# rsjahnige/CRYSTALS-Kyber

Hardware: NVIDIA B200
Metric: ML-KEM-768 Encaps+Decaps ops/s (higher is better)
Workload: dtype u16/u64 integer

## Files before the change

crystals-kyber_b200/csrc/mlkem_b200.cu:

```cuda
#include "mlkem_kernels.cuh"

#include "../../include/mlkem_b200.h"

#include <algorithm>
#include <atomic>
#include <cstdio>
#include <cstdlib>
#include <cstring>
#include <mutex>
#include <vector>

namespace {

using namespace mlkem;

thread_local char tl_error[512] = "";
std::atomic<unsigned long long> g_launches{0};
int env_int(const char *name, int dflt) {
    const char *v = getenv(name);
    return v && *v ? atoi(v) : dflt;
}
constexpr int kSlots = 6;
constexpr int kDevSlots = 4;
constexpr int kHostSlots = 3;
constexpr int kMaxDevices = 64;
int initial_streams() {
    int v = env_int("MLKEM_B200_STREAMS", 0);
    return v < 1 ? kDevSlots : (v > kDevSlots ? kDevSlots : v);
}
std::atomic<int> g_streams{initial_streams()};
int warp_hash_max() {
    static const int v = env_int("MLKEM_B200_WARP_HASH_MAX", kWarpHashMaxItems);
    return v;
}

#define CU(call)                                                                                              \
    do {                                                                                                      \
        cudaError_t e_ = (call);                                                                              \
        if (e_ != cudaSuccess) {                                                                              \
            snprintf(tl_error, sizeof tl_error, "%s failed: %s (%s:%d)", #call, cudaGetErrorString(e_), __FILE__, __LINE__); \
            return MLKEM_B200_ERR_CUDA;                                                                       \
        }                                                                                                     \
    } while (0)

struct ProfEntry {
    const char *name;
    cudaEvent_t e0, e1;
};
std::atomic<int> g_profile{0};
std::mutex g_prof_mutex;
std::vector<ProfEntry> g_prof_entries;

inline void prof_begin(const char *name, cudaStream_t st, ProfEntry &pe, bool &on) {
    on = g_profile.load(std::memory_order_relaxed) != 0;
    if (!on) return;
    pe.name = name;
    cudaEventCreate(&pe.e0);
    cudaEventCreate(&pe.e1);
    cudaEventRecord(pe.e0, st);
}
inline void prof_end(cudaStream_t st, ProfEntry &pe, bool on) {
    if (!on) return;
    cudaEventRecord(pe.e1, st);
    std::lock_guard<std::mutex> lock(g_prof_mutex);
    g_prof_entries.push_back(pe);
}

#define LAUNCH(kernel, grid, block, smem, stream, ...)           \
    do {                                                         \
        auto kern_ = kernel;                                     \
        ProfEntry pe_;                                           \
        bool prof_on_;                                           \
        prof_begin(#kernel, (stream), pe_, prof_on_);            \
        kern_<<<(grid), (block), (smem), (stream)>>>(__VA_ARGS__); \
        prof_end((stream), pe_, prof_on_);                       \
        g_launches.fetch_add(1, std::memory_order_relaxed);      \
        CU(cudaGetLastError());                                  \
    } while (0)

inline unsigned cdiv(size_t a, size_t b) { return (unsigned)((a + b - 1) / b); }
inline unsigned warp_hash_grid(int n) { return cdiv((size_t)n, kWarpHashTPB / 32); }
inline unsigned warp_grid(size_t items, int warps_per_block) {
    size_t blocks = (items + warps_per_block - 1) / warps_per_block;
    const size_t cap = 148 * 16;
    return (unsigned)(blocks < cap ? blocks : cap);
}

unsigned bitrev7(unsigned r) {
    unsigned o = 0;
    for (int i = 0; i < 7; i++) o |= ((r >> i) & 1u) << (6 - i);
    return o;
}
unsigned pow17(unsigned e) {
    unsigned z = 1;
    while (e--) z = (z * 17u) % kQ;
    return z;
}
uint2 shoup_pair(unsigned w) { return make_uint2(w, (w << 16) / kQ); }
uint2 shoup_pair32(unsigned w) { return make_uint2(w, (unsigned)(((unsigned long long)w << 32) / kQ)); }

void build_tables(TwiddleTables &t, uint2 rc[24]) {
    for (unsigned i = 0; i < 128; i++) {
        t.zeta[i] = shoup_pair(pow17(bitrev7(i)));
        t.gamma[i] = shoup_pair(pow17(2 * bitrev7(i) + 1));
        t.gamma32[i] = shoup_pair32(t.gamma[i].x);
        t.zeta32[i] = shoup_pair32(t.zeta[i].x);
    }
    t.zeta_inv_last[0] = shoup_pair((t.zeta[1].x * 3303u) % kQ);
    t.zeta_inv_last[1] = shoup_pair(3303u);
    t.zeta_inv_last32[0] = shoup_pair32(t.zeta_inv_last[0].x);
    t.zeta_inv_last32[1] = shoup_pair32(3303u);
    uint8_t lfsr = 1;
    for (int round = 0; round < 24; round++) {
        unsigned long long c = 0;
        for (int j = 0; j <= 6; j++) {
            if (lfsr & 1) c |= 1ULL << ((1u << j) - 1);
            uint8_t hi = lfsr & 0x80;
            lfsr = (uint8_t)(lfsr << 1);
            if (hi) lfsr ^= 0x71;
        }
        rc[round] = make_uint2((unsigned)c, (unsigned)(c >> 32));
    }
}

struct DeviceCtx {
    bool ready = false;
    cudaStream_t stream[kSlots] = {};
    void *ws[kSlots] = {};
    size_t ws_bytes[kSlots] = {};
    void *io[kSlots] = {};
    size_t io_bytes[kSlots] = {};
    cudaEvent_t ev_fork = nullptr, ev_join[kSlots] = {}, ev_slot[kSlots] = {};
    void *misc = nullptr;
    size_t misc_bytes = 0;
    int host_group = 0;
    std::mutex call_mutex;
    std::mutex misc_mutex;
};
DeviceCtx g_ctx[kMaxDevices];
std::mutex g_mutex;

struct DeviceGuard {
    int prev = -1;
    bool changed = false;
    int enter(int d) {
        if (cudaGetDevice(&prev) != cudaSuccess) prev = -1;
        if (prev == d) return 0;
        CU(cudaSetDevice(d));
        changed = true;
        return 0;
    }
    ~DeviceGuard() {
        if (changed && prev >= 0) cudaSetDevice(prev);
    }
};

int ensure_buffer(void **p, size_t *have, size_t need, cudaEvent_t last_use = nullptr) {
    if (*have >= need) return 0;
    if (*p) {
        if (last_use) CU(cudaEventSynchronize(last_use));
        CU(cudaMemset(*p, 0, *have));
        CU(cudaFree(*p));
    }
    *p = nullptr;
    *have = 0;
    size_t want = need + need / 8;
    CU(cudaMalloc(p, want));
    *have = want;
    return 0;
}

template <class KernelT>
int allow_smem(KernelT kernel, size_t bytes) {
    CU(cudaFuncSetAttribute(kernel, cudaFuncAttributeMaxDynamicSharedMemorySize, (int)bytes));
    CU(cudaFuncSetAttribute(kernel, cudaFuncAttributePreferredSharedMemoryCarveout, cudaSharedmemCarveoutMaxShared));
    return 0;
}
template <class P>
int allow_smem_matvec() {
    const size_t b = matvec_smem_bytes<P>();
    if (int rc = allow_smem(k_sample_matvec<P, kModeKeyGen>, b)) return rc;
    if (int rc = allow_smem(k_sample_matvec<P, kModeEncrypt>, b)) return rc;
    if (int rc = allow_smem(k_sample_matvec<P, kModeEncryptCompare>, b)) return rc;
    if (int rc = allow_smem(k_sample_matvec_list<P, kModeKeyGen>, b)) return rc;
    if (int rc = allow_smem(k_sample_matvec_list<P, kModeEncrypt>, b)) return rc;
    if (int rc = allow_smem(k_sample_matvec_list<P, kModeEncryptCompare>, b)) return rc;
    return 0;
}

int acquire(const mlkem_b200_opts *o, int *dev, DeviceCtx **ctx, DeviceGuard &guard) {
    int d = o ? o->device : -1;
    if (d < 0) CU(cudaGetDevice(&d));
    if (d >= kMaxDevices) {
        snprintf(tl_error, sizeof tl_error, "device ordinal %d out of range", d);
        return MLKEM_B200_ERR_ARG;
    }
    if (int rc = guard.enter(d)) return rc;
    std::lock_guard<std::mutex> lock(g_mutex);
    DeviceCtx &c = g_ctx[d];
    if (!c.ready) {
        cudaStream_t st[kSlots] = {};
        cudaEvent_t ev[2 * kSlots + 1] = {};
        auto create = [&]() -> int {
            TwiddleTables t;
            uint2 rc[24];
            build_tables(t, rc);
            CU(cudaMemcpyToSymbol(c_tw, &t, sizeof t));
            CU(cudaMemcpyToSymbol(g_tw, &t, sizeof t));
            CU(cudaMemcpyToSymbol(c_keccak_rc, rc, sizeof rc));
            uint32_t pow2[32];
            for (int k = 0; k < 32; k++) pow2[k] = 1u << k;
            CU(cudaMemcpyToSymbol(c_pow2, pow2, sizeof pow2));
            for (int s = 0; s < kSlots; s++) CU(cudaStreamCreateWithFlags(&st[s], cudaStreamNonBlocking));
            for (int e = 0; e < 2 * kSlots + 1; e++) CU(cudaEventCreateWithFlags(&ev[e], cudaEventDisableTiming));
            if (int r = allow_smem_matvec<P512>()) return r;
            if (int r = allow_smem_matvec<P768>()) return r;
            if (int r = allow_smem_matvec<P1024>()) return r;
            if (int r = allow_smem(k_sample_ntt_batch, 128 * kSlotWords * 4)) return r;
            return 0;
        };
        if (int r = create()) {
            for (auto s_ : st)
                if (s_) cudaStreamDestroy(s_);
            for (auto e_ : ev)
                if (e_) cudaEventDestroy(e_);
            return r;
        }
        for (int s = 0; s < kSlots; s++) {
            c.stream[s] = st[s];
            c.ev_join[s] = ev[s];
            c.ev_slot[s] = ev[kSlots + s];
        }
        c.ev_fork = ev[2 * kSlots];
        c.ready = true;
    }
    *dev = d;
    *ctx = &c;
    return 0;
}

struct Arena {
    uint8_t *base;
    size_t off = 0;
    explicit Arena(void *p) : base(static_cast<uint8_t *>(p)) {}
    template <class T>
    T *take(size_t count) {
        off = (off + 255) & ~size_t(255);
        T *p = reinterpret_cast<T *>(base + off);
        off += count * sizeof(T);
        return p;
    }
};

template <class P>
constexpr size_t ws_bytes_per_item() {
    size_t kg = 64 + 2 * P::K * 512 + 4 * P::K;
    size_t enc = P::K * 512 + (P::K + 1) * 128 + 32 + 4 * P::K;
    size_t dec = enc + 32 + 64 + 4;
    size_t m = kg > dec ? kg : dec;
    return m + 64;
}
constexpr size_t kWsSlack = 16 * 256;


template <class P, int MODE>
int launch_matvec(cudaStream_t st, Arena &ws, MatvecArgs a) {
    constexpr int K = P::K;
    const size_t rows = (size_t)a.n * K, smem = matvec_smem_bytes<P>();
    const unsigned blocks = cdiv(rows, 32), list_grid = std::min<unsigned>(blocks, 148 * 4);
#ifdef MLKEM_B200_EXPERIMENT
    static const int env_exp = env_int("MLKEM_B200_EXPERIMENT", 0);
    a.experiment = env_exp;
#endif
    if (a.group_limit >= 168 && rows > 32) {
        a.defer_list = ws.take<int>(rows);
        a.defer_count = ws.take<int>(1);
        CU(cudaMemsetAsync(a.defer_count, 0, sizeof(int), st));
        LAUNCH((k_sample_matvec<P, MODE>), blocks, 32 * K, smem, st, a);
#ifdef MLKEM_B200_EXPERIMENT
        if (env_exp & 16) return 0;
#endif
        LAUNCH((k_sample_matvec_list<P, MODE>), list_grid, 32 * K, smem, st, a);
    } else {
        a.defer_list = nullptr;
        a.defer_count = nullptr;
        LAUNCH((k_sample_matvec_list<P, MODE>), list_grid, 32 * K, smem, st, a);
    }
    return 0;
}

template <class P>
int enqueue_encrypt(cudaStream_t st, Arena &ws, int n, const uint8_t *ek, size_t ek_stride, KeySel keys, const uint8_t *m,
                    const uint8_t *seed, size_t seed_stride, uint8_t *c, const uint8_t *cmp, uint32_t *flags, int group_limit, bool fips,
                    const uint16_t *matrix = nullptr) {
    constexpr int K = P::K;
    uint16_t *yhat = ws.take<uint16_t>((size_t)n * K * 256);
    uint32_t *codes = ws.take<uint32_t>((size_t)n * (K + 1) * 32);
    if (!fips) {
        LAUNCH((k_noise<P::ETA1, true>), dim3(cdiv(n, kNoiseTPB), K), kNoiseTPB, 0, st, n, seed, seed_stride, 0, yhat, (size_t)K * 256,
               (uint32_t *)nullptr, (size_t)0, (uint8_t *)nullptr, (size_t)0, 0);
        LAUNCH((k_noise<P::ETA2, false>), dim3(cdiv(n, kNoiseTPB), K + 1), kNoiseTPB, 0, st, n, seed, seed_stride, K, (uint16_t *)nullptr,
               (size_t)0, codes, (size_t)(K + 1) * 32, (uint8_t *)nullptr, (size_t)0, 0);
    } else {
        LAUNCH((k_noise<P::ETA1, true, kRateSha3_256>), dim3(cdiv(n, kNoiseTPB), K), kNoiseTPB, 0, st, n, seed, seed_stride, 0, yhat,
               (size_t)K * 256, (uint32_t *)nullptr, (size_t)0, (uint8_t *)nullptr, (size_t)0, 0);
        LAUNCH((k_noise<P::ETA2, false, kRateSha3_256>), dim3(cdiv(n, kNoiseTPB), K + 1), kNoiseTPB, 0, st, n, seed, seed_stride, K,
               (uint16_t *)nullptr, (size_t)0, codes, (size_t)(K + 1) * 32, (uint8_t *)nullptr, (size_t)0, 0);
    }
    MatvecArgs a{};
    a.n = n;
    a.group_limit = group_limit;
    a.rho = ek + 384 * K;
    a.rho_stride = ek_stride;
    a.keys = keys;
    a.vec = yhat;
    a.vec_stride = (size_t)K * 256;
    a.addc = codes;
    a.addc_stride = (size_t)(K + 1) * 32;
    a.out = c;
    a.out_stride = P::C;
    a.cmp = cmp;
    a.flags = flags;
    EncVArgs v{};
    v.n = n;
    v.ek = ek;
    v.ek_stride = ek_stride;
    v.keys = keys;
    v.yhat = yhat;
    v.yhat_stride = (size_t)K * 256;
    v.addc = codes;
    v.addc_stride = (size_t)(K + 1) * 32;
    v.m = m;
    v.c = c;
    v.c_stride = P::C;
    v.cmp = cmp;
    v.flags = flags;
    const unsigned tgrid = warp_grid((size_t)n * K, kMatTableTPB / 32);
    if (cmp) {
        if (matrix) LAUNCH((k_matvec_table<P, kModeEncryptCompare>), tgrid, kMatTableTPB, 0, st, a, matrix);
        else if (int rc = launch_matvec<P, kModeEncryptCompare>(st, ws, a)) return rc;
        LAUNCH((k_encrypt_v<P, true>), warp_grid(n, kWarpTPB / 32), kWarpTPB, 0, st, v);
    } else {
        if (matrix) LAUNCH((k_matvec_table<P, kModeEncrypt>), tgrid, kMatTableTPB, 0, st, a, matrix);
        else if (int rc = launch_matvec<P, kModeEncrypt>(st, ws, a)) return rc;
        LAUNCH((k_encrypt_v<P, false>), warp_grid(n, kWarpTPB / 32), kWarpTPB, 0, st, v);
    }
    return 0;
}

template <class P>
int enqueue_keygen(cudaStream_t st, Arena &ws, int n, const uint8_t *d, const uint8_t *z, uint8_t *ek, uint8_t *dk, int group_limit, bool fips) {
    constexpr int K = P::K;
    const bool full = z != nullptr;
    const size_t dk_stride = full ? P::DK : P::DKPKE;
    uint8_t *rs = ws.take<uint8_t>((size_t)n * 64);
    uint16_t *se = ws.take<uint16_t>((size_t)n * 2 * K * 256);
    LAUNCH(k_keygen_G, cdiv(n, kHashTPB), kHashTPB, 0, st, n, d, (uint32_t)K, rs, ek + 384 * K, (size_t)P::EK,
           full ? dk + 768 * K : (uint8_t *)nullptr, dk_stride);
    if (!fips)
        LAUNCH((k_noise<P::ETA1, true>), dim3(cdiv(n, kNoiseTPB), 2 * K), kNoiseTPB, 0, st, n, rs + 32, (size_t)64, 0, se, (size_t)2 * K * 256,
               (uint32_t *)nullptr, (size_t)0, dk, dk_stride, K);
    else
        LAUNCH((k_noise<P::ETA1, true, kRateSha3_256>), dim3(cdiv(n, kNoiseTPB), 2 * K), kNoiseTPB, 0, st, n, rs + 32, (size_t)64, 0, se,
               (size_t)2 * K * 256, (uint32_t *)nullptr, (size_t)0, dk, dk_stride, K);
    MatvecArgs a{};
    a.n = n;
    a.group_limit = group_limit;
    a.rho = rs;
    a.rho_stride = 64;
    a.vec = se;
    a.vec_stride = (size_t)2 * K * 256;
    a.add16 = se + K * 256;
    a.add16_stride = (size_t)2 * K * 256;
    a.out = ek;
    a.out_stride = P::EK;
    a.out2 = full ? dk + 384 * K : nullptr;
    a.out2_stride = dk_stride;
    if (int rc = launch_matvec<P, kModeKeyGen>(st, ws, a)) return rc;
    if (full && n <= warp_hash_max()) LAUNCH((k_keygen_H_warp<P>), warp_hash_grid(n), kWarpHashTPB, 0, st, n, ek, z, dk);
    else if (full) LAUNCH((k_keygen_H<P>), cdiv(n, kHashTPB), kHashTPB, 0, st, n, ek, z, dk);
    return 0;
}

template <class P>
int enqueue_encaps(cudaStream_t st, Arena &ws, int n, const uint8_t *ek, const uint8_t *m, uint8_t *c, uint8_t *Kout, int group_limit, bool fips) {
    uint8_t *r = ws.take<uint8_t>((size_t)n * 32);
    if (n <= warp_hash_max()) LAUNCH((k_encaps_HG_warp<P>), warp_hash_grid(n), kWarpHashTPB, 0, st, n, ek, m, Kout, r);
    else LAUNCH((k_encaps_HG<P>), cdiv(n, kHashTPB), kHashTPB, 0, st, n, ek, m, Kout, r);
    return enqueue_encrypt<P>(st, ws, n, ek, P::EK, KeySel{}, m, r, 32, c, nullptr, nullptr, group_limit, fips);
}

template <class P>
int enqueue_encaps_keyed(cudaStream_t st, Arena &ws, int n, const uint8_t *ek, size_t ek_stride, const uint8_t *hek, KeySel keys,
                         const uint8_t *m, uint8_t *c, uint8_t *Kout, int group_limit, bool fips, const uint16_t *matrix) {
    uint8_t *r = ws.take<uint8_t>((size_t)n * 32);
    LAUNCH(k_encaps_G_keyed, cdiv(n, kHashTPB), kHashTPB, 0, st, n, hek, keys, m, Kout, r);
    return enqueue_encrypt<P>(st, ws, n, ek, ek_stride, keys, m, r, 32, c, nullptr, nullptr, group_limit, fips, matrix);
}

template <class P>
int enqueue_decaps(cudaStream_t st, Arena &ws, int n, const uint8_t *dk, KeySel keys, const uint8_t *c, uint8_t *Kout, int group_limit, bool fips,
                   const uint16_t *matrix = nullptr) {
    constexpr int K = P::K;
    uint8_t *mp = ws.take<uint8_t>((size_t)n * 32);
    uint8_t *Kr = ws.take<uint8_t>((size_t)n * 64);
    uint32_t *flags = ws.take<uint32_t>((size_t)n);
    CU(cudaMemsetAsync(flags, 0, (size_t)n * 4, st));
    LAUNCH((k_decrypt<P>), warp_grid(n, kWarpTPB / 32), kWarpTPB, 0, st, n, dk, (size_t)P::DK, keys, c, mp);
    LAUNCH((k_decaps_G<P>), cdiv(n, kHashTPB), kHashTPB, 0, st, n, mp, dk, keys, Kr);
    if (int rc = enqueue_encrypt<P>(st, ws, n, dk + 384 * K, P::DK, keys, mp, Kr + 32, 64, nullptr, c, flags, group_limit, fips, matrix)) return rc;
    if (n <= warp_hash_max()) {
        if (!fips) LAUNCH((k_decaps_J_select_warp<P>), warp_hash_grid(n), kWarpHashTPB, 0, st, n, dk, keys, c, Kr, flags, Kout);
        else LAUNCH((k_decaps_J_select_warp<P, kRateSha3_256>), warp_hash_grid(n), kWarpHashTPB, 0, st, n, dk, keys, c, Kr, flags, Kout);
        return 0;
    }
    if (!fips) LAUNCH((k_decaps_J_select<P>), cdiv(n, kHashTPB), kHashTPB, 0, st, n, dk, keys, c, Kr, flags, Kout);
    else LAUNCH((k_decaps_J_select<P, kRateSha3_256>), cdiv(n, kHashTPB), kHashTPB, 0, st, n, dk, keys, c, Kr, flags, Kout);
    return 0;
}

struct Buf {
    const void *in;
    void *out;
    size_t item_bytes;
    bool cells = false;
};

int launch_narrow(cudaStream_t st, const void *cells, void *dense, size_t bytes) {
    const size_t nw = bytes / 4;
    if (nw) LAUNCH(k_cells_to_bytes, cdiv(nw, 256), 256, 0, st, nw, (const uint4 *)cells, (uint32_t *)dense);
    return 0;
}
int launch_widen(cudaStream_t st, const void *dense, void *cells, size_t bytes) {
    const size_t nw = bytes / 4;
    if (nw) LAUNCH(k_bytes_to_cells, cdiv(nw, 256), 256, 0, st, nw, (const uint32_t *)dense, (uint4 *)cells);
    return 0;
}

bool aligned16(const void *p) { return (reinterpret_cast<uintptr_t>(p) & 15) == 0; }

template <class Run>
int drive(const mlkem_b200_opts *o, size_t n, size_t ws_per_item, std::vector<Buf> bufs, Run run) {
    if (n == 0) return MLKEM_B200_OK;
    if (n > 0x7FFFFFFFull / 8) {
        snprintf(tl_error, sizeof tl_error, "batch too large");
        return MLKEM_B200_ERR_ARG;
    }
    for (auto &b : bufs)
        if (!b.in && !b.out) {
            snprintf(tl_error, sizeof tl_error, "NULL buffer");
            return MLKEM_B200_ERR_ARG;
        }
    int dev;
    DeviceCtx *ctx;
    DeviceGuard guard;
    if (int rc = acquire(o, &dev, &ctx, guard)) return rc;
    std::unique_lock<std::mutex> call_lock(ctx->call_mutex);
    const bool on_device = o && o->mem == MLKEM_B200_MEM_DEVICE;
    static const int env_chunk = env_int("MLKEM_B200_CHUNK", 0);
    static const int env_hchunk = env_int("MLKEM_B200_HOST_CHUNK", 0);
    static const int host_slots = std::min(kHostSlots, std::max(1, env_int("MLKEM_B200_HOST_SLOTS", kHostSlots)));
    size_t chunk = (o && o->chunk_items > 0) ? (size_t)o->chunk_items
                   : (on_device ? (env_chunk > 0 ? (size_t)env_chunk : (size_t)1 << 18) : (env_hchunk > 0 ? (size_t)env_hchunk : (size_t)1 << 16));
    if (chunk > ((size_t)1 << 26)) chunk = (size_t)1 << 26;
    if (chunk > n) chunk = n;
    const size_t nchunks = (n + chunk - 1) / chunk;
    std::vector<void *> ptrs(bufs.size());
    size_t cell_dense_per_item = 0;
    for (auto &b : bufs)
        if (b.cells) cell_dense_per_item += (b.item_bytes + 15) & ~size_t(15);

    if (on_device) {
        for (auto &b : bufs)
            if (!aligned16(b.in ? b.in : b.out)) {
                snprintf(tl_error, sizeof tl_error, "device pointers must be 16-byte aligned");
                return MLKEM_B200_ERR_ARG;
            }
        cudaStream_t st = static_cast<cudaStream_t>(o->stream);
        if (!(o && o->chunk_items > 0) && n >= ((size_t)1 << 16) && nchunks < 2 && g_streams.load() > 1) {
            chunk = ((n + 1) / 2 + 1023) & ~(size_t)1023;
        }
        const size_t nch = (n + chunk - 1) / chunk;
        int nstreams = g_streams.load();
        if (nstreams > kDevSlots) nstreams = kDevSlots;
        if ((size_t)nstreams > nch) nstreams = (int)nch;
        if (nstreams < 1) nstreams = 1;
        {
            std::lock_guard<std::mutex> lock(g_mutex);
            for (int k = 0; k < nstreams; k++)
                if (int rc = ensure_buffer(&ctx->ws[k], &ctx->ws_bytes[k], chunk * (ws_per_item + cell_dense_per_item) + kWsSlack + 256 * bufs.size(),
                                           ctx->ev_slot[k]))
                    return rc;
        }
        const bool fork = nstreams > 1;
        if (fork) CU(cudaEventRecord(ctx->ev_fork, st));
        for (int k = 0; k < nstreams; k++) {
            cudaStream_t sk = fork ? ctx->stream[k] : st;
            if (fork) CU(cudaStreamWaitEvent(sk, ctx->ev_fork, 0));
            CU(cudaStreamWaitEvent(sk, ctx->ev_slot[k], 0));
        }
        int rc = 0;
        for (size_t ci = 0; ci < nch && !rc; ci++) {
            size_t i0 = ci * chunk, cn = (i0 + chunk <= n) ? chunk : n - i0;
            const int k = fork ? (int)(ci % nstreams) : 0;
            cudaStream_t sk = fork ? ctx->stream[k] : st;
            Arena arena(ctx->ws[k]);
            for (size_t b = 0; b < bufs.size() && !rc; b++) {
                const uint8_t *base = static_cast<const uint8_t *>(bufs[b].in ? bufs[b].in : bufs[b].out);
                if (!bufs[b].cells) {
                    ptrs[b] = const_cast<uint8_t *>(base) + i0 * bufs[b].item_bytes;
                } else {
                    ptrs[b] = arena.take<uint8_t>(cn * bufs[b].item_bytes);
// ... 1187 lines not shown
```

crystals-kyber_b200/csrc/mlkem_device.cuh:

```cuda
#pragma once
#include <cuda_runtime.h>
#include <stdint.h>

namespace mlkem {

constexpr int kN = 256;
constexpr uint32_t kQ = 3329;
constexpr uint32_t kFullMask = 0xFFFFFFFFu;

struct TwiddleTables {
    uint2 zeta[128];
    uint2 zeta_inv_last[2];
    uint2 gamma[128];
    uint2 gamma32[128];
    uint2 zeta32[128];
    uint2 zeta_inv_last32[2];
};
__constant__ TwiddleTables c_tw;
__device__ TwiddleTables g_tw;
__constant__ uint2 c_keccak_rc[24];
__constant__ uint32_t c_pow2[32];
__device__ __forceinline__ uint32_t shl_fma(uint32_t x, int k) { return x * c_pow2[k]; }
__device__ __forceinline__ uint2 lane_zeta(int i) { return __ldg(&g_tw.zeta[i]); }
__device__ __forceinline__ uint2 lane_zeta32(int i) { return __ldg(&g_tw.zeta32[i]); }
__device__ __forceinline__ uint2 lane_gamma(int i) { return __ldg(&g_tw.gamma32[i]); }


__device__ __forceinline__ uint32_t mulhi(uint32_t a, uint32_t b) {
#ifndef MLKEM_B200_MULHI_WIDE
    return __umulhi(a, b);
#else
    [[maybe_unused]] uint32_t lo;
    uint32_t hi;
    asm volatile("{.reg .b64 t; mul.wide.u32 t, %2, %3; mov.b64 {%0, %1}, t;}" : "=r"(lo), "=r"(hi) : "r"(a), "r"(b));
    return hi;
#endif
}

__device__ __forceinline__ uint32_t mul_shoup(uint32_t a, uint2 w) {
    uint32_t qh = (a * w.y) >> 16;
    return a * w.x - qh * kQ;
}
__device__ __forceinline__ uint32_t mul_shoup_fma(uint32_t a, uint32_t w, uint32_t w32) {
    uint32_t qh = mulhi(a, w32);
    return a * w - qh * kQ;
}
constexpr bool kFmaPipe = true, kBalanced = false;
template <bool FMA>
__device__ __forceinline__ uint32_t mulz(uint32_t a, uint2 z) {
    return FMA ? mul_shoup_fma(a, z.x, z.y) : mul_shoup(a, z);
}
__device__ __forceinline__ uint32_t canon_fma(uint32_t x) { return x - mulhi(x, 1290168u) * kQ; }
__device__ __forceinline__ uint32_t barrett16(uint32_t x) {
    uint32_t qh = (x * 40317u) >> 27;
    return x - qh * kQ;
}
__device__ __forceinline__ uint32_t barrett32(uint32_t x) {
    uint32_t qh = mulhi(x, 1290167u);
    return x - qh * kQ;
}
__device__ __forceinline__ uint32_t csubq(uint32_t r) { return min(r, r - kQ); }
__device__ __forceinline__ uint32_t canon16(uint32_t x) { return csubq(barrett16(x)); }
__device__ __forceinline__ uint32_t canon32(uint32_t x) { return csubq(barrett32(x)); }

template <int D>
__device__ __forceinline__ uint32_t compress(uint32_t x) {
    if (D >= 12) return x;
    uint32_t t = (x << D) + 1664u;
    uint32_t qh = mulhi(t, 1290167u);
    uint32_t r = t - qh * kQ;
    qh += (r >= kQ);
    return qh & ((1u << D) - 1u);
}
template <int D>
__device__ __forceinline__ uint32_t compress_canon(uint32_t x) {
    static_assert(D == 1 || D == 4 || D == 5 || D == 10 || D == 11, "no verified constants for this d");
    constexpr uint32_t c = (D >= 10) ? 1664u : 1665u, M = (D >= 10) ? 1290168u : 1290167u;
    return mulhi(x * (1u << D) + c, M) & ((1u << D) - 1u);
}

template <int D>
__device__ __forceinline__ uint32_t compress_resid(uint32_t x) {
    static_assert(D == 1 || D == 4 || D == 5, "single multiply-high is not exact on residues for this d");
    return mulhi(x * (1u << D) + 1664u, 1290168u) & ((1u << D) - 1u);
}

template <int D>
__device__ __forceinline__ uint32_t decompress(uint32_t y) {
    if (D >= 12) return y;
    return (kQ * y + (1u << (D - 1))) >> D;
}

struct Lane {
    uint32_t lo, hi;
};

template <int R>
__device__ __forceinline__ Lane rotl64(Lane x) {
    Lane r = x;
    if constexpr (R == 32) {
        r.lo = x.hi;
        r.hi = x.lo;
    } else if constexpr (R > 0 && R < 32) {
        r.hi = __funnelshift_l(x.lo, x.hi, R);
        r.lo = __funnelshift_l(x.hi, x.lo, R);
    } else if constexpr (R > 32) {
        r.hi = __funnelshift_l(x.hi, x.lo, R - 32);
        r.lo = __funnelshift_l(x.lo, x.hi, R - 32);
    }
    return r;
}
__device__ __forceinline__ Lane xor3(Lane a, Lane b, Lane c) { return Lane{a.lo ^ b.lo ^ c.lo, a.hi ^ b.hi ^ c.hi}; }
__device__ __forceinline__ Lane xor5(Lane a, Lane b, Lane c, Lane d, Lane e) {
    return Lane{a.lo ^ b.lo ^ c.lo ^ d.lo ^ e.lo, a.hi ^ b.hi ^ c.hi ^ d.hi ^ e.hi};
}
__device__ __forceinline__ Lane chi3(Lane a, Lane b, Lane c) { return Lane{a.lo ^ (~b.lo & c.lo), a.hi ^ (~b.hi & c.hi)}; }

__device__ __forceinline__ void keccak_f1600(Lane a[25]) {
#pragma unroll 2
    for (int rnd = 0; rnd < 24; rnd++) {
        Lane c0 = xor5(a[0], a[5], a[10], a[15], a[20]), c1 = xor5(a[1], a[6], a[11], a[16], a[21]),
             c2 = xor5(a[2], a[7], a[12], a[17], a[22]), c3 = xor5(a[3], a[8], a[13], a[18], a[23]),
             c4 = xor5(a[4], a[9], a[14], a[19], a[24]);
        Lane r0 = rotl64<1>(c0), r1 = rotl64<1>(c1), r2 = rotl64<1>(c2), r3 = rotl64<1>(c3), r4 = rotl64<1>(c4);
#define MLKEM_TH(x, cm, rp)             \
    a[x] = xor3(a[x], cm, rp);          \
    a[x + 5] = xor3(a[x + 5], cm, rp);  \
    a[x + 10] = xor3(a[x + 10], cm, rp); \
    a[x + 15] = xor3(a[x + 15], cm, rp); \
    a[x + 20] = xor3(a[x + 20], cm, rp);
        MLKEM_TH(0, c4, r1) MLKEM_TH(1, c0, r2) MLKEM_TH(2, c1, r3) MLKEM_TH(3, c2, r4) MLKEM_TH(4, c3, r0)
#undef MLKEM_TH
        Lane b[25];
        b[0] = a[0];             b[10] = rotl64<1>(a[1]);   b[20] = rotl64<62>(a[2]);  b[5] = rotl64<28>(a[3]);   b[15] = rotl64<27>(a[4]);
        b[16] = rotl64<36>(a[5]); b[1] = rotl64<44>(a[6]);   b[11] = rotl64<6>(a[7]);   b[21] = rotl64<55>(a[8]);  b[6] = rotl64<20>(a[9]);
        b[7] = rotl64<3>(a[10]);  b[17] = rotl64<10>(a[11]); b[2] = rotl64<43>(a[12]);  b[12] = rotl64<25>(a[13]); b[22] = rotl64<39>(a[14]);
        b[23] = rotl64<41>(a[15]); b[8] = rotl64<45>(a[16]); b[18] = rotl64<15>(a[17]); b[3] = rotl64<21>(a[18]);  b[13] = rotl64<8>(a[19]);
        b[14] = rotl64<18>(a[20]); b[24] = rotl64<2>(a[21]); b[9] = rotl64<61>(a[22]);  b[19] = rotl64<56>(a[23]); b[4] = rotl64<14>(a[24]);
#pragma unroll
        for (int y = 0; y < 25; y += 5) {
#pragma unroll
            for (int x = 0; x < 5; x++) a[y + x] = chi3(b[y + x], b[y + (x + 1) % 5], b[y + (x + 2) % 5]);
        }
        uint2 rc = c_keccak_rc[rnd];
        a[0].lo ^= rc.x;
        a[0].hi ^= rc.y;
    }
}

__device__ __forceinline__ void keccak_zero(Lane a[25]) {
#pragma unroll
    for (int i = 0; i < 25; i++) a[i] = Lane{0u, 0u};
}

constexpr uint32_t kSfxHash = 0x06;
constexpr uint32_t kSfxXof = 0x1F;
constexpr int kRateShake128 = 21;
constexpr int kRateSha3_256 = 17;
constexpr int kRateSha3_512 = 9;

template <int RATE, typename F>
__device__ __forceinline__ void sponge_absorb_words(Lane a[25], int nwords, uint32_t sfx, F word) {
    keccak_zero(a);
    int base = 0;
    for (; base + RATE <= nwords; base += RATE) {
#pragma unroll
        for (int i = 0; i < RATE; i++) {
            Lane w = word(base + i);
            a[i].lo ^= w.lo;
            a[i].hi ^= w.hi;
        }
        keccak_f1600(a);
    }
    int rem = nwords - base;
#pragma unroll
    for (int i = 0; i < RATE; i++) {
        if (i < rem) {
            Lane w = word(base + i);
            a[i].lo ^= w.lo;
            a[i].hi ^= w.hi;
        } else if (i == rem) {
            a[i].lo ^= sfx;
        }
    }
    a[RATE - 1].hi ^= 0x80000000u;
    keccak_f1600(a);
}

__device__ __forceinline__ Lane load_lane(const uint8_t *p) {
    uint2 v = *reinterpret_cast<const uint2 *>(p);
    return Lane{v.x, v.y};
}
__device__ __forceinline__ void store_lane(uint8_t *p, Lane v) { *reinterpret_cast<uint2 *>(p) = make_uint2(v.lo, v.hi); }

struct WarpSponge {
    int s5, s10, s15, s20;
    int xm, xp;
    int pi;
    int c1, c2;
    uint32_t shift;
    bool swap, first;
};
__device__ __forceinline__ WarpSponge warp_sponge_init(int lane) {
    constexpr uint32_t kRho[7] = {0u | 1u << 8 | 62u << 16 | 28u << 24,  27u | 36u << 8 | 44u << 16 | 6u << 24,  55u | 20u << 8 | 3u << 16 | 10u << 24,
                                  43u | 25u << 8 | 39u << 16 | 41u << 24, 45u | 15u << 8 | 21u << 16 | 8u << 24, 18u | 2u << 8 | 61u << 16 | 56u << 24,
                                  14u};
    WarpSponge w;
    const bool act = lane < 25;
    const int x = lane % 5, y = lane / 5;
    w.s5 = act ? (lane + 5) % 25 : lane;
    w.s10 = act ? (lane + 10) % 25 : lane;
    w.s15 = act ? (lane + 15) % 25 : lane;
    w.s20 = act ? (lane + 20) % 25 : lane;
    w.xm = act ? (x + 4) % 5 : lane;
    w.xp = act ? (x + 1) % 5 : lane;
    w.pi = act ? (x + 3 * y) % 5 + 5 * x : lane;
    w.c1 = act ? 5 * y + (x + 1) % 5 : lane;
    w.c2 = act ? 5 * y + (x + 2) % 5 : lane;
    uint32_t word = 0;
#pragma unroll
    for (int k = 0; k < 7; k++) word = (lane >> 2) == k ? kRho[k] : word;
    const uint32_t rot = act ? (word >> (8 * (lane & 3))) & 63u : 0u;
    w.shift = rot & 31u;
    w.swap = (rot & 32u) != 0;
    w.first = lane == 0;
    return w;
}
__device__ __forceinline__ Lane shfl_lane(Lane v, int src) {
    return Lane{__shfl_sync(kFullMask, v.lo, src), __shfl_sync(kFullMask, v.hi, src)};
}
__device__ __forceinline__ void keccak_f1600_warp(Lane &a, const WarpSponge &w) {
#pragma unroll 2
    for (int rnd = 0; rnd < 24; rnd++) {
        const Lane c = xor5(a, shfl_lane(a, w.s5), shfl_lane(a, w.s10), shfl_lane(a, w.s15), shfl_lane(a, w.s20));
        a = xor3(a, shfl_lane(c, w.xm), rotl64<1>(shfl_lane(c, w.xp)));
        const uint32_t lo = w.swap ? a.hi : a.lo, hi = w.swap ? a.lo : a.hi;
        a.hi = __funnelshift_l(lo, hi, w.shift);
        a.lo = __funnelshift_l(hi, lo, w.shift);
        const Lane b = shfl_lane(a, w.pi);
        a = chi3(b, shfl_lane(b, w.c1), shfl_lane(b, w.c2));
        const uint2 rc = c_keccak_rc[rnd];
        a.lo ^= w.first ? rc.x : 0u;
        a.hi ^= w.first ? rc.y : 0u;
    }
}
template <int RATE, typename F>
__device__ __forceinline__ Lane warp_sponge_absorb_words(int lane, const WarpSponge &w, int nwords, uint32_t sfx, F word) {
    Lane a{0u, 0u};
    int base = 0;
    for (; base + RATE <= nwords; base += RATE) {
        if (lane < RATE) {
            const Lane v = word(base + lane);
            a.lo ^= v.lo;
            a.hi ^= v.hi;
        }
        keccak_f1600_warp(a, w);
    }
    const int rem = nwords - base;
    if (lane < rem) {
        const Lane v = word(base + lane);
        a.lo ^= v.lo;
        a.hi ^= v.hi;
    } else if (lane == rem) {
        a.lo ^= sfx;
    }
    if (lane == RATE - 1) a.hi ^= 0x80000000u;
    keccak_f1600_warp(a, w);
    return a;
}

constexpr int kScratchU16 = 256;
__device__ __forceinline__ int sidx(int c) { return c ^ (((c >> 6) & 3) << 3); }
__device__ __forceinline__ int idxA(int lane, int r) { return lane + 32 * r; }
__device__ __forceinline__ int idxB(int lane, int r) { return ((lane >> 2) << 5) | (r << 2) | (lane & 3); }
__device__ __forceinline__ int idxC(int lane, int r) { return 8 * lane + r; }

struct LaneTwiddles {
    uint2 z16;
    uint2 z8[2];
    uint2 z4[4];
    uint2 z2[2];
};
template <bool FMA = false>
__device__ __forceinline__ uint2 lane_z(int i) { return FMA ? lane_zeta32(i) : lane_zeta(i); }
template <bool FMA = false>
__device__ __forceinline__ uint2 uniform_z(int i) { return FMA ? c_tw.zeta32[i] : c_tw.zeta[i]; }
template <bool FMA = false>
__device__ __forceinline__ void load_lane_twiddles(LaneTwiddles &t, int lane) {
    int g = lane >> 2;
    t.z16 = lane_z<FMA>(8 + g);
#pragma unroll
    for (int i = 0; i < 2; i++) t.z8[i] = lane_z<FMA>(16 + 2 * g + i);
#pragma unroll
    for (int i = 0; i < 4; i++) t.z4[i] = lane_z<FMA>(32 + 4 * g + i);
#pragma unroll
    for (int i = 0; i < 2; i++) t.z2[i] = lane_z<FMA>(64 + 2 * lane + i);
}
template <bool FMA = false>
__device__ __forceinline__ void load_lane_twiddles_inv(LaneTwiddles &t, int lane) {
    int g = lane >> 2;
    t.z16 = lane_z<FMA>(15 - g);
#pragma unroll
    for (int i = 0; i < 2; i++) t.z8[i] = lane_z<FMA>(31 - (2 * g + i));
#pragma unroll
    for (int i = 0; i < 4; i++) t.z4[i] = lane_z<FMA>(63 - (4 * g + i));
#pragma unroll
    for (int i = 0; i < 2; i++) t.z2[i] = lane_z<FMA>(127 - (2 * lane + i));
}

__device__ __forceinline__ void store_scratch_A(const uint32_t x[8], uint16_t *s, int lane) {
#pragma unroll
    for (int r = 0; r < 8; r++) s[sidx(idxA(lane, r))] = (uint16_t)x[r];
}
__device__ __forceinline__ void load_scratch_A(uint32_t x[8], const uint16_t *s, int lane) {
#pragma unroll
    for (int r = 0; r < 8; r++) x[r] = s[sidx(idxA(lane, r))];
}
__device__ __forceinline__ void store_scratch_B(const uint32_t x[8], uint16_t *s, int lane) {
#pragma unroll
    for (int r = 0; r < 8; r++) s[sidx(idxB(lane, r))] = (uint16_t)x[r];
}
__device__ __forceinline__ void load_scratch_B(uint32_t x[8], const uint16_t *s, int lane) {
#pragma unroll
    for (int r = 0; r < 8; r++) x[r] = s[sidx(idxB(lane, r))];
}
__device__ __forceinline__ uint4 pack_pairs(const uint32_t x[8]) {
    return make_uint4(x[0] + x[1] * 65536u, x[2] + x[3] * 65536u, x[4] + x[5] * 65536u, x[6] + x[7] * 65536u);
}
__device__ __forceinline__ void unpack_pairs(uint4 v, uint32_t x[8]) {
    x[0] = v.x & 0xFFFFu; x[1] = v.x >> 16; x[2] = v.y & 0xFFFFu; x[3] = v.y >> 16;
    x[4] = v.z & 0xFFFFu; x[5] = v.z >> 16; x[6] = v.w & 0xFFFFu; x[7] = v.w >> 16;
}
__device__ __forceinline__ void store_scratch_C(const uint32_t x[8], uint16_t *s, int lane) {
    *reinterpret_cast<uint4 *>(s + sidx(8 * lane)) = pack_pairs(x);
}
__device__ __forceinline__ void load_scratch_C(uint32_t x[8], const uint16_t *s, int lane) {
    unpack_pairs(*reinterpret_cast<const uint4 *>(s + sidx(8 * lane)), x);
}

template <bool FMA = false>
__device__ __forceinline__ void ct_bfly(uint32_t &a, uint32_t &b, uint2 z) {
    uint32_t t = mulz<FMA>(b, z);
    b = a - t + 2 * kQ;
    a = a + t;
}

template <bool FMA = false>
__device__ __forceinline__ void ntt_warp(uint32_t x[8], uint16_t *scratch, int lane, const LaneTwiddles &tw) {
#pragma unroll
    for (int r = 0; r < 4; r++) ct_bfly<FMA>(x[r], x[r + 4], uniform_z<FMA>(1));
#pragma unroll
    for (int h = 0; h < 2; h++)
#pragma unroll
        for (int r = 0; r < 2; r++) ct_bfly<FMA>(x[4 * h + r], x[4 * h + r + 2], uniform_z<FMA>(2 + h));
#pragma unroll
    for (int h = 0; h < 4; h++) ct_bfly<FMA>(x[2 * h], x[2 * h + 1], uniform_z<FMA>(4 + h));
    store_scratch_A(x, scratch, lane);
    __syncwarp();
    load_scratch_B(x, scratch, lane);
    __syncwarp();
#pragma unroll
    for (int r = 0; r < 4; r++) ct_bfly<FMA>(x[r], x[r + 4], tw.z16);
#pragma unroll
    for (int h = 0; h < 2; h++)
#pragma unroll
        for (int r = 0; r < 2; r++) ct_bfly<FMA>(x[4 * h + r], x[4 * h + r + 2], tw.z8[h]);
#pragma unroll
    for (int h = 0; h < 4; h++) ct_bfly<FMA>(x[2 * h], x[2 * h + 1], tw.z4[h]);
    store_scratch_B(x, scratch, lane);
    __syncwarp();
    load_scratch_C(x, scratch, lane);
    __syncwarp();
#pragma unroll
    for (int h = 0; h < 2; h++)
#pragma unroll
        for (int r = 0; r < 2; r++) ct_bfly<FMA>(x[4 * h + r], x[4 * h + r + 2], tw.z2[h]);
#pragma unroll
    for (int r = 0; r < 8; r++) x[r] = FMA ? canon_fma(x[r]) : canon16(x[r]);
}

__device__ __forceinline__ void ct_bfly_exact(uint32_t &a, uint32_t &b, uint2 z) {
    const uint32_t t = csubq(mul_shoup(b, z)), lo = a;
    b = lo >= t ? lo - t : kQ - (t - lo);
    a = canon16(lo + t);
}
__device__ __forceinline__ void ntt_warp_exact(uint32_t x[8], uint16_t *scratch, int lane) {
    LaneTwiddles tw;
    load_lane_twiddles<false>(tw, lane);
#pragma unroll
    for (int r = 0; r < 4; r++) ct_bfly_exact(x[r], x[r + 4], uniform_z<false>(1));
#pragma unroll
    for (int h = 0; h < 2; h++)
#pragma unroll
        for (int r = 0; r < 2; r++) ct_bfly_exact(x[4 * h + r], x[4 * h + r + 2], uniform_z<false>(2 + h));
#pragma unroll
    for (int h = 0; h < 4; h++) ct_bfly_exact(x[2 * h], x[2 * h + 1], uniform_z<false>(4 + h));
    store_scratch_A(x, scratch, lane);
    __syncwarp();
    load_scratch_B(x, scratch, lane);
    __syncwarp();
#pragma unroll
    for (int r = 0; r < 4; r++) ct_bfly_exact(x[r], x[r + 4], tw.z16);
#pragma unroll
    for (int h = 0; h < 2; h++)
#pragma unroll
        for (int r = 0; r < 2; r++) ct_bfly_exact(x[4 * h + r], x[4 * h + r + 2], tw.z8[h]);
#pragma unroll
    for (int h = 0; h < 4; h++) ct_bfly_exact(x[2 * h], x[2 * h + 1], tw.z4[h]);
    store_scratch_B(x, scratch, lane);
    __syncwarp();
    load_scratch_C(x, scratch, lane);
    __syncwarp();
#pragma unroll
    for (int h = 0; h < 2; h++)
#pragma unroll
        for (int r = 0; r < 2; r++) ct_bfly_exact(x[4 * h + r], x[4 * h + r + 2], tw.z2[h]);
}

template <bool FMA = false>
__device__ __forceinline__ void gs_bfly(uint32_t &a, uint32_t &b, uint2 z, uint32_t bias) {
    uint32_t t = a;
    a = t + b;
    b = mulz<FMA>(b - t + bias, z);
}

template <bool FMA = false, bool CANON = true>
__device__ __forceinline__ void intt_warp(uint32_t x[8], uint16_t *scratch, int lane, const LaneTwiddles &tw) {
#pragma unroll
    for (int h = 0; h < 2; h++)
#pragma unroll
        for (int r = 0; r < 2; r++) gs_bfly<FMA>(x[4 * h + r], x[4 * h + r + 2], tw.z2[h], (FMA ? 3 : 2) * kQ);
    store_scratch_C(x, scratch, lane);
    __syncwarp();
    load_scratch_B(x, scratch, lane);
    __syncwarp();
#pragma unroll
    for (int h = 0; h < 4; h++) {
        gs_bfly<FMA>(x[2 * h], x[2 * h + 1], tw.z4[h], (FMA ? 5 : 3) * kQ);
        x[2 * h] = FMA ? barrett32(x[2 * h]) : barrett16(x[2 * h]);
    }
#pragma unroll
    for (int h = 0; h < 2; h++)
#pragma unroll
        for (int r = 0; r < 2; r++) gs_bfly<FMA>(x[4 * h + r], x[4 * h + r + 2], tw.z8[h], 2 * kQ);
#pragma unroll
    for (int r = 0; r < 4; r++) gs_bfly<FMA>(x[r], x[r + 4], tw.z16, 4 * kQ);
    store_scratch_B(x, scratch, lane);
    __syncwarp();
    load_scratch_A(x, scratch, lane);
    __syncwarp();
#pragma unroll
    for (int h = 0; h < 4; h++) {
        gs_bfly<FMA>(x[2 * h], x[2 * h + 1], uniform_z<FMA>(7 - h), 8 * kQ);
        x[2 * h] = FMA ? barrett32(x[2 * h]) : barrett16(x[2 * h]);
    }
#pragma unroll
    for (int h = 0; h < 2; h++)
#pragma unroll
        for (int r = 0; r < 2; r++) gs_bfly<FMA>(x[4 * h + r], x[4 * h + r + 2], uniform_z<FMA>(3 - h), 2 * kQ);
    const uint2 zs = FMA ? c_tw.zeta_inv_last32[1] : c_tw.zeta_inv_last[1], zl = FMA ? c_tw.zeta_inv_last32[0] : c_tw.zeta_inv_last[0];
#pragma unroll
    for (int r = 0; r < 4; r++) {
        uint32_t t = x[r];
        x[r] = mulz<FMA>(t + x[r + 4], zs);
        x[r + 4] = mulz<FMA>(x[r + 4] - t + 4 * kQ, zl);
        if (CANON) {
            x[r] = csubq(x[r]);
            x[r + 4] = csubq(x[r + 4]);
        }
    }
}

__device__ __forceinline__ void basemul_acc(uint32_t &acc0, uint32_t &acc1, uint32_t a0, uint32_t a1, uint32_t b0,
                                            uint32_t b1, uint2 gamma) {
    uint32_t a1g = mul_shoup_fma(a1, gamma.x, gamma.y);
    acc0 += a0 * b0 + a1g * b1;
    acc1 += a0 * b1 + a1 * b0;
}

template <int D>
__device__ __forceinline__ void pack8(const uint32_t v[8], uint8_t *dst) {
    constexpr int NW = (8 * D + 31) / 32;
    uint32_t w[NW];
#pragma unroll
    for (int k = 0; k < NW; k++) {
        uint32_t acc = 0;
#pragma unroll
        for (int i = 0; i < 8; i++) {
            const int off = D * i - 32 * k;
            if (off >= 0 && off < 32) acc += v[i] * (1u << off);
            else if (off < 0 && off + D > 0) acc += v[i] >> (-off);
        }
        w[k] = acc;
    }
    if (D % 4 == 0) {
#pragma unroll
        for (int k = 0; k < NW; k++) reinterpret_cast<uint32_t *>(dst)[k] = w[k];
    } else if (D % 2 == 0) {
#pragma unroll
        for (int h = 0; h < D / 2; h++) reinterpret_cast<uint16_t *>(dst)[h] = (uint16_t)(w[h >> 1] >> (16 * (h & 1)));
    } else {
#pragma unroll
        for (int b8 = 0; b8 < D; b8++) dst[b8] = (uint8_t)(w[b8 >> 2] >> (8 * (b8 & 3)));
    }
}
template <int D>
__device__ __forceinline__ void unpack8(const uint8_t *row, int lane, uint32_t v[8]) {
    const uint32_t *w = reinterpret_cast<const uint32_t *>(row);
    const int bit = 8 * D * lane, wi = bit >> 5, s = bit & 31;
    constexpr int NA = (8 * D + 31) / 32;
    uint32_t raw[NA + 1], a[NA + 1];
#pragma unroll
    for (int k = 0; k <= NA; k++) raw[k] = ((8 * D) % 32 == 0 && k == NA) ? 0u : w[wi + k];
#pragma unroll
    for (int k = 0; k < NA; k++) a[k] = ((8 * D) % 32 == 0) ? raw[k] : __funnelshift_r(raw[k], raw[k + 1], s);
    a[NA] = 0;
#pragma unroll
    for (int i = 0; i < 8; i++) {
        const int o = D * i, k = o >> 5, sh = o & 31;
        uint32_t f = (sh + D <= 32) ? (a[k] >> sh) : __funnelshift_r(a[k], a[k + 1], sh);
        v[i] = f & ((1u << D) - 1u);
    }
}

template <int D>
__device__ __forceinline__ uint32_t unpack1(const uint8_t *src, int c) {
    if (D == 1) return (src[c >> 3] >> (c & 7)) & 1u;
    if (D == 4) return (src[c >> 1] >> ((c & 1) * 4)) & 15u;
    const int bit = D * c, byte = bit >> 3, sh = bit & 7;
    uint32_t w = (uint32_t)src[byte];
    if (sh + D > 8) w |= (uint32_t)src[byte + 1] << 8;
    if (D > 9 && sh + D > 16) w |= (uint32_t)src[byte + 2] << 16;
    return (w >> sh) & ((1u << D) - 1u);
}

template <int S>
__device__ __forceinline__ uint32_t shr_fma(uint32_t x) {
    return mulhi(x, 1u << (32 - S));
}
#ifndef MLKEM_B200_NIBBLE_ALU
__device__ __forceinline__ uint32_t nibble_fma(uint32_t w, uint32_t sel) { return shr_fma<28>(w * sel); }
__device__ __forceinline__ uint32_t nibble_weight(int j) { return 1u << (28 - 4 * j); }
#else
__device__ __forceinline__ uint32_t nibble_fma(uint32_t w, uint32_t sel) { return (w >> sel) & 15u; }
__device__ __forceinline__ uint32_t nibble_weight(int j) { return 4 * j; }
#endif

__device__ __forceinline__ uint32_t noise_code_to_coeff(uint32_t code) {
    return csubq(code + (kQ - 3));
}
__device__ __forceinline__ uint32_t add_noise_code(uint32_t x, uint32_t code) {
    return csubq(csubq(x + code + (kQ - 3)));
}

}
```

crystals-kyber_b200/csrc/mlkem_kernels.cuh:

```cuda
#pragma once
#include "mlkem_device.cuh"

namespace mlkem {

template <int K_, int ETA1_, int ETA2_, int DU_, int DV_>
struct ParamSet {
    static constexpr int K = K_, ETA1 = ETA1_, ETA2 = ETA2_, DU = DU_, DV = DV_;
    static constexpr int EK = 384 * K + 32;
    static constexpr int DKPKE = 384 * K;
    static constexpr int DK = 768 * K + 96;
    static constexpr int C1ROW = 32 * DU;
    static constexpr int C2 = 32 * DV;
    static constexpr int C = C1ROW * K + C2;
};
using P512 = ParamSet<2, 3, 2, 10, 4>;
using P768 = ParamSet<3, 2, 2, 10, 4>;
using P1024 = ParamSet<4, 2, 2, 11, 5>;

struct KeySel {
    const uint32_t *index;
    uint32_t base, nkeys;
};
__device__ __forceinline__ size_t key_row(const KeySel &k, int item) {
    if (k.index) return min(__ldg(k.index + item), k.nkeys - 1u);
// ... 115 lines not shown
__global__ void __launch_bounds__(kHashTPB) k_hash_ek_table(int n, const uint8_t *__restrict__ ek, size_t ek_stride, uint8_t *__restrict__ hek) {
    int i = blockIdx.x * blockDim.x + threadIdx.x;
    if (i >= n) return;
    Lane h[4];
    hash_H_ek<P>(ek + ek_stride * i, h);
#pragma unroll
    for (int w = 0; w < 4; w++) store_lane(hek + 32 * (size_t)i + 8 * w, h[w]);
}

template <class P>
__global__ void __launch_bounds__(kHashTPB) k_check_dk_hash(int n, const uint8_t *__restrict__ dk, int *__restrict__ status) {
    int i = blockIdx.x * blockDim.x + threadIdx.x;
    if (i >= n) return;
    const uint8_t *base = dk + (size_t)P::DK * i;
    Lane h[4];
    hash_H_ek<P>(base + 384 * P::K, h);
    uint32_t diff = 0;
#pragma unroll
    for (int w = 0; w < 4; w++) {
        Lane s = load_lane(base + 768 * P::K + 32 + 8 * w);
        diff |= (s.lo ^ h[w].lo) | (s.hi ^ h[w].hi);
    }
    status[i] = diff ? -5 : 0;
}

template <class P>
__global__ void __launch_bounds__(kHashTPB) k_check_ek_modulus(int n, const uint8_t *__restrict__ ek, int *__restrict__ status) {
    int i = blockIdx.x * blockDim.x + threadIdx.x;
    if (i >= n) return;
    const uint32_t *w = reinterpret_cast<const uint32_t *>(ek + (size_t)P::EK * i);
    uint32_t bad = 0;
    for (int t = 0; t < 96 * P::K; t += 3) {
        uint32_t w0 = __ldg(w + t), w1 = __ldg(w + t + 1), w2 = __ldg(w + t + 2);
        uint32_t c[8] = {w0 & 0xFFF, (w0 >> 12) & 0xFFF, (w0 >> 24) | ((w1 & 0xF) << 8), (w1 >> 4) & 0xFFF,
                         (w1 >> 16) & 0xFFF, (w1 >> 28) | ((w2 & 0xFF) << 4), (w2 >> 8) & 0xFFF, w2 >> 20};
#pragma unroll
        for (int k = 0; k < 8; k++) bad |= (c[k] >= kQ);
    }
    status[i] = bad ? -4 : 0;
}

__global__ void __launch_bounds__(kHashTPB) k_mask_keys(int n, const int *__restrict__ status, uint8_t *__restrict__ K) {
    int i = blockIdx.x * blockDim.x + threadIdx.x;
    if (i >= n) return;
    if (status[i] != 0) {
        uint4 zero = make_uint4(0, 0, 0, 0);
        reinterpret_cast<uint4 *>(K + 32 * (size_t)i)[0] = zero;
        reinterpret_cast<uint4 *>(K + 32 * (size_t)i)[1] = zero;
    }
}

template <class P>
__global__ void __launch_bounds__(kHashTPB) k_decaps_G(int n, const uint8_t *__restrict__ mprime, const uint8_t *__restrict__ dk, KeySel keys,
                                                       uint8_t *__restrict__ Kr) {
    int i = blockIdx.x * blockDim.x + threadIdx.x;
    if (i >= n) return;
    Lane h[4], mm[4], a[25];
    const uint8_t *hp = dk + (size_t)P::DK * key_row(keys, i) + 768 * P::K + 32;
#pragma unroll
    for (int w = 0; w < 4; w++) {
        mm[w] = load_lane(mprime + 32 * (size_t)i + 8 * w);
        h[w] = load_lane(hp + 8 * w);
    }
    hash_G_64(a, mm, h);
#pragma unroll
    for (int w = 0; w < 8; w++) store_lane(Kr + 64 * (size_t)i + 8 * w, a[w]);
}

template <class P, int RATE = kRateShake128>
__global__ void __launch_bounds__(kHashTPB) k_decaps_J_select(int n, const uint8_t *__restrict__ dk, KeySel keys, const uint8_t *__restrict__ c,
                                                              const uint8_t *__restrict__ Kr, const uint32_t *__restrict__ flags,
                                                              uint8_t *__restrict__ Kout) {
    int i = blockIdx.x * blockDim.x + threadIdx.x;
    if (i >= n) return;
    const uint8_t *z = dk + (size_t)P::DK * key_row(keys, i) + 768 * P::K + 64;
    const uint8_t *ci = c + (size_t)P::C * i;
    Lane a[25];
    sponge_absorb_words<RATE>(a, 4 + P::C / 8, kSfxXof,
                              [&](int w) { return w < 4 ? load_lane(z + 8 * w) : load_lane(ci + 8 * (w - 4)); });
    uint32_t mask = flags[i] ? 0xFFFFFFFFu : 0u;
#pragma unroll
    for (int w = 0; w < 4; w++) {
        Lane kp = load_lane(Kr + 64 * (size_t)i + 8 * w);
        Lane o{(a[w].lo & mask) | (kp.lo & ~mask), (a[w].hi & mask) | (kp.hi & ~mask)};
        store_lane(Kout + 32 * (size_t)i + 8 * w, o);
    }
}

constexpr int kWarpHashTPB = 128;
constexpr int kWarpHashMaxItems = 1024;

template <class P>
__device__ __forceinline__ Lane warp_hash_H_ek(const uint8_t *ek, int lane, const WarpSponge &w) {
    return warp_sponge_absorb_words<kRateSha3_256>(lane, w, P::EK / 8, kSfxHash, [&](int i) { return load_lane(ek + 8 * i); });
}
__device__ __forceinline__ Lane warp_hash_G_64(const uint8_t *x, Lane y03, int lane, const WarpSponge &w) {
    const Lane y = shfl_lane(y03, (lane - 4) & 31);
    Lane a{0u, 0u};
    if (lane < 4) a = load_lane(x + 8 * lane);
    else if (lane < 8) a = y;
    else if (lane == 8) a = Lane{kSfxHash, 0x80000000u};
    keccak_f1600_warp(a, w);
    return a;
}

template <class P>
__global__ void __launch_bounds__(kWarpHashTPB) k_keygen_H_warp(int n, const uint8_t *__restrict__ ek, const uint8_t *__restrict__ z,
                                                                uint8_t *__restrict__ dk) {
    const int lane = threadIdx.x & 31, i = blockIdx.x * (kWarpHashTPB / 32) + (threadIdx.x >> 5);
    if (i >= n) return;
    const WarpSponge w = warp_sponge_init(lane);
    const Lane h = warp_hash_H_ek<P>(ek + (size_t)P::EK * i, lane, w);
    uint8_t *tail = dk + (size_t)P::DK * i + 768 * P::K + 32;
    if (lane < 4) store_lane(tail + 8 * lane, h);
    else if (lane < 8) store_lane(tail + 8 * lane, load_lane(z + 32 * (size_t)i + 8 * (lane - 4)));
}

template <class P>
__global__ void __launch_bounds__(kWarpHashTPB) k_encaps_HG_warp(int n, const uint8_t *__restrict__ ek, const uint8_t *__restrict__ m,
                                                                 uint8_t *__restrict__ Kout, uint8_t *__restrict__ r) {
    const int lane = threadIdx.x & 31, i = blockIdx.x * (kWarpHashTPB / 32) + (threadIdx.x >> 5);
    if (i >= n) return;
    const WarpSponge w = warp_sponge_init(lane);
    const Lane h = warp_hash_H_ek<P>(ek + (size_t)P::EK * i, lane, w);
    const Lane a = warp_hash_G_64(m + 32 * (size_t)i, h, lane, w);
    if (lane < 4) store_lane(Kout + 32 * (size_t)i + 8 * lane, a);
    else if (lane < 8) store_lane(r + 32 * (size_t)i + 8 * (lane - 4), a);
}

template <class P>
__global__ void __launch_bounds__(kWarpHashTPB) k_check_dk_hash_warp(int n, const uint8_t *__restrict__ dk, int *__restrict__ status) {
    const int lane = threadIdx.x & 31, i = blockIdx.x * (kWarpHashTPB / 32) + (threadIdx.x >> 5);
    if (i >= n) return;
    const WarpSponge w = warp_sponge_init(lane);
    const uint8_t *base = dk + (size_t)P::DK * i;
    const Lane h = warp_hash_H_ek<P>(base + 384 * P::K, lane, w);
    bool diff = false;
    if (lane < 4) {
        const Lane s = load_lane(base + 768 * P::K + 32 + 8 * lane);
        diff = ((s.lo ^ h.lo) | (s.hi ^ h.hi)) != 0;
    }
    const bool any = __any_sync(kFullMask, diff);
    if (lane == 0) status[i] = any ? -5 : 0;
}

template <class P, int RATE = kRateShake128>
__global__ void __launch_bounds__(kWarpHashTPB) k_decaps_J_select_warp(int n, const uint8_t *__restrict__ dk, KeySel keys, const uint8_t *__restrict__ c,
                                                                       const uint8_t *__restrict__ Kr, const uint32_t *__restrict__ flags,
                                                                       uint8_t *__restrict__ Kout) {
    const int lane = threadIdx.x & 31, i = blockIdx.x * (kWarpHashTPB / 32) + (threadIdx.x >> 5);
    if (i >= n) return;
    const WarpSponge w = warp_sponge_init(lane);
    const uint8_t *z = dk + (size_t)P::DK * key_row(keys, i) + 768 * P::K + 64;
    const uint8_t *ci = c + (size_t)P::C * i;
    const Lane a = warp_sponge_absorb_words<RATE>(lane, w, 4 + P::C / 8, kSfxXof,
                                                  [&](int t) { return t < 4 ? load_lane(z + 8 * t) : load_lane(ci + 8 * (t - 4)); });
    const uint32_t mask = flags[i] ? 0xFFFFFFFFu : 0u;
    if (lane < 4) {
        const Lane kp = load_lane(Kr + 64 * (size_t)i + 8 * lane);
        store_lane(Kout + 32 * (size_t)i + 8 * lane, Lane{(a.lo & mask) | (kp.lo & ~mask), (a.hi & mask) | (kp.hi & ~mask)});
    }
}

template <int RATE, int OUTW>
__global__ void __launch_bounds__(kHashTPB) k_hash_words(int n, const uint8_t *__restrict__ in, int nwords, uint32_t sfx,
                                                         uint8_t *__restrict__ out) {
    int i = blockIdx.x * blockDim.x + threadIdx.x;
    if (i >= n) return;
    const uint8_t *p = in + (size_t)nwords * 8 * i;
    Lane a[25];
    sponge_absorb_words<RATE>(a, nwords, sfx, [&](int w) { return load_lane(p + 8 * w); });
#pragma unroll
    for (int w = 0; w < OUTW; w++) store_lane(out + (size_t)OUTW * 8 * i + 8 * w, a[w]);
}

__global__ void __launch_bounds__(kHashTPB) k_sponge_padded(int n, const uint8_t *__restrict__ padded, int nblocks, int rl,
                                                            uint8_t *__restrict__ out, int out_bytes) {
    int i = blockIdx.x * blockDim.x + threadIdx.x;
    if (i >= n) return;
    const uint8_t *p = padded + (size_t)i * nblocks * rl * 8;
    Lane a[25];
    keccak_zero(a);
    for (int b = 0; b < nblocks; b++) {
#pragma unroll
        for (int l = 0; l < 25; l++)
            if (l < rl) {
                Lane w = load_lane(p + ((size_t)b * rl + l) * 8);
                a[l].lo ^= w.lo;
                a[l].hi ^= w.hi;
            }
        keccak_f1600(a);
    }
    const int out_stride = (out_bytes + 7) & ~7;
    uint8_t *o = out + (size_t)i * out_stride;
    int done = 0;
    while (done < out_bytes) {
        int take = min(rl * 8, out_bytes - done);
#pragma unroll
        for (int l = 0; l < 25; l++)
            if (l * 8 < take) store_lane(o + done + l * 8, a[l]);
        done += take;
        if (done < out_bytes) keccak_f1600(a);
    }
}


__device__ __forceinline__ uint32_t cbd2_word(uint32_t w) {
    uint32_t t = w - ((w >> 1) & 0x55555555u);
    uint32_t x = t & 0x33333333u, y = (t >> 2) & 0x33333333u;
    return x + (0x33333333u - y);
}
__device__ __forceinline__ uint32_t cbd3_chunk(uint32_t c24) {
    uint32_t t = (c24 & 0x249249u) + ((c24 >> 1) & 0x249249u) + ((c24 >> 2) & 0x249249u);
    uint32_t out = 0;
#pragma unroll
    for (int m = 0; m < 4; m++) {
        uint32_t x = (t >> (6 * m)) & 7u, y = (t >> (6 * m + 3)) & 7u;
        out |= (x + 3u - y) << (4 * m);
    }
    return out;
}
__device__ __forceinline__ void cbd3_words(uint32_t w0, uint32_t w1, uint32_t w2, uint32_t &o0, uint32_t &o1) {
    uint32_t c0 = w0 & 0xFFFFFFu, c1 = (w0 >> 24) | ((w1 & 0xFFFFu) << 8), c2 = (w1 >> 16) | ((w2 & 0xFFu) << 16), c3 = w2 >> 8;
    o0 = cbd3_chunk(c0) | (cbd3_chunk(c1) << 16);
    o1 = cbd3_chunk(c2) | (cbd3_chunk(c3) << 16);
}

template <int ETA, int RATE, typename PUT>
__device__ __forceinline__ void prf_cbd_codes(const Lane seed[4], uint32_t nonce, PUT put) {
    Lane a[25];
    keccak_zero(a);
#pragma unroll
    for (int w = 0; w < 4; w++) a[w] = seed[w];
    a[4].lo = nonce | (kSfxXof << 8);
    a[RATE - 1].hi ^= 0x80000000u;
    keccak_f1600(a);
    if (ETA == 2) {
#pragma unroll
        for (int l = 0; l < 16; l++) {
            put(2 * l, cbd2_word(a[l].lo));
            put(2 * l + 1, cbd2_word(a[l].hi));
        }
    } else {
        constexpr int W1 = 2 * RATE;
        constexpr int G1 = W1 / 3;
        uint32_t o0, o1;
#pragma unroll
        for (int g = 0; g < G1; g++) {
            const int w = 3 * g;
            uint32_t w0 = (w & 1) ? a[w >> 1].hi : a[w >> 1].lo, w1 = ((w + 1) & 1) ? a[(w + 1) >> 1].hi : a[(w + 1) >> 1].lo,
                     w2 = ((w + 2) & 1) ? a[(w + 2) >> 1].hi : a[(w + 2) >> 1].lo;
            cbd3_words(w0, w1, w2, o0, o1);
            put(2 * g, o0);
            put(2 * g + 1, o1);
        }
        constexpr int LEFT = W1 - 3 * G1;
        uint32_t carry = 0;
        if (LEFT) carry = ((W1 - 1) & 1) ? a[(W1 - 1) >> 1].hi : a[(W1 - 1) >> 1].lo;
        keccak_f1600(a);
        int next = 0;
        if (LEFT) {
            cbd3_words(carry, a[0].lo, a[0].hi, o0, o1);
            put(2 * G1, o0);
            put(2 * G1 + 1, o1);
            next = 2;
        }
#pragma unroll
        for (int g = G1 + (LEFT ? 1 : 0); g < 16; g++) {
            const int w = next + 3 * (g - G1 - (LEFT ? 1 : 0));
            uint32_t w0 = (w & 1) ? a[w >> 1].hi : a[w >> 1].lo, w1 = ((w + 1) & 1) ? a[(w + 1) >> 1].hi : a[(w + 1) >> 1].lo,
                     w2 = ((w + 2) & 1) ? a[(w + 2) >> 1].hi : a[(w + 2) >> 1].lo;
            cbd3_words(w0, w1, w2, o0, o1);
            put(2 * g, o0);
            put(2 * g + 1, o1);
        }
    }
}

__device__ __forceinline__ void store_layoutC_global(const uint32_t x[8], int lane, uint16_t *dst) {
    reinterpret_cast<uint4 *>(dst)[lane] = pack_pairs(x);
}
__device__ __forceinline__ void load_layoutC_global(uint32_t x[8], int lane, const uint16_t *src) {
    unpack_pairs(__ldg(reinterpret_cast<const uint4 *>(src) + lane), x);
}

template <int ETA, bool NTT_OUT, int RATE = kRateShake128>
__global__ void __launch_bounds__(kNoiseTPB) k_noise(int n, const uint8_t *__restrict__ seeds, size_t seed_stride, int nonce0,
                                                     uint16_t *__restrict__ out16, size_t out16_stride,
                                                     uint32_t *__restrict__ outc, size_t outc_stride,
                                                     uint8_t *__restrict__ enc12, size_t enc12_stride, int enc12_polys) {
    __shared__ uint32_t s_codes[NTT_OUT ? kNoiseTPB * 33 : 1];
    __shared__ __align__(16) uint16_t s_scratch[NTT_OUT ? (kNoiseTPB / 32) * kScratchU16 : 2];
    const int p = blockIdx.y;
    const int item = blockIdx.x * kNoiseTPB + threadIdx.x;
    Lane seed[4];
#pragma unroll
    for (int w = 0; w < 4; w++) seed[w] = item < n ? load_lane(seeds + seed_stride * item + 8 * w) : Lane{0u, 0u};
    if (NTT_OUT) {
        uint32_t *mine = s_codes + 33 * threadIdx.x;
        prf_cbd_codes<ETA, RATE>(seed, (uint32_t)(nonce0 + p), [&](int w, uint32_t v) { mine[w] = v; });
        __syncwarp();
        const int lane = threadIdx.x & 31, warp = threadIdx.x >> 5;
        uint16_t *scratch = s_scratch + warp * kScratchU16;
        LaneTwiddles tw;
        load_lane_twiddles<kFmaPipe>(tw, lane);
        const uint32_t pw = nibble_weight(lane & 7);
        for (int t = 0; t < 32; t++) {
            int it = blockIdx.x * kNoiseTPB + warp * 32 + t;
            if (it >= n) break;
            const uint32_t *codes = s_codes + 33 * (warp * 32 + t) + (lane >> 3);
            uint32_t x[8];
#pragma unroll
            for (int r = 0; r < 8; r++) x[r] = nibble_fma(codes[4 * r], pw) + (kQ - 3);
            ntt_warp<kFmaPipe>(x, scratch, lane, tw);
            store_layoutC_global(x, lane, out16 + out16_stride * it + 256 * p);
            if (p < enc12_polys) {
                uint32_t *row = reinterpret_cast<uint32_t *>(enc12 + enc12_stride * it + 384 * p) + 3 * lane;
                row[0] = x[0] | (x[1] << 12) | (x[2] << 24);
                row[1] = (x[2] >> 8) | (x[3] << 4) | (x[4] << 16) | (x[5] << 28);
                row[2] = (x[5] >> 4) | (x[6] << 8) | (x[7] << 20);
            }
        }
    } else {
        if (item >= n) return;
        uint32_t buf[32];
        prf_cbd_codes<ETA, RATE>(seed, (uint32_t)(nonce0 + p), [&](int w, uint32_t v) { buf[w] = v; });
        uint4 *dst = reinterpret_cast<uint4 *>(outc + outc_stride * item + 32 * p);
#pragma unroll
        for (int v = 0; v < 8; v++) dst[v] = make_uint4(buf[4 * v], buf[4 * v + 1], buf[4 * v + 2], buf[4 * v + 3]);
    }
}

template <bool CHECKED>
__device__ __forceinline__ void parse_block(const Lane a[25], uint32_t &addr, uint32_t end_addr) {
#pragma unroll
    for (int ch = 0; ch < 7; ch++) {
        const uint32_t w[7] = {a[3 * ch].lo, a[3 * ch].hi, a[3 * ch + 1].lo, a[3 * ch + 1].hi, a[3 * ch + 2].lo, a[3 * ch + 2].hi, 0u};
#pragma unroll
        for (int m = 0; m < 16; m++) {
            const int bit = 12 * m, wi = bit >> 5, sh = bit & 31;
            uint32_t t;
            if (sh == 20) t = w[wi];
            else if (sh < 20) t = w[wi] * (1u << (20 - sh));
            else t = __funnelshift_r(w[wi], w[wi + 1], sh - 20);
            bool ok = t < (kQ << 20);
            if (CHECKED) ok = ok && (addr < end_addr);
            uint32_t d;
            asm("mul.hi.u32 %0, %1, 4096;" : "=r"(d) : "r"(t));
            if (ok) {
                asm volatile("st.shared.u16 [%0], %1;" ::"r"(addr), "h"((uint16_t)d) : "memory");
                addr += 2;
            }
        }
    }
}

__device__ __forceinline__ void mask_groups(Lane a[25], int usable) {
    const int cut = 24 * max(usable, 0);
#pragma unroll
    for (int k = 0; k < 42; k++) {
        const int lo = 32 * k;
        uint32_t m = cut <= lo ? 0xFFFFFFFFu : (cut >= lo + 32 ? 0u : (0xFFFFFFFFu << (cut - lo)));
        if (k & 1) a[k >> 1].hi |= m;
        else a[k >> 1].lo |= m;
    }
}

__device__ __forceinline__ void sample_ntt_thread(const Lane rho[4], uint32_t &b32, uint32_t &b33, uint16_t *slot, bool active,
                                                  int group_limit) {
    Lane a[25];
    const uint32_t base = (uint32_t)__cvta_generic_to_shared(slot), end_addr = base + 2 * kN;
    uint32_t addr = active ? base : end_addr;
    int groups_left = 0;
    bool need_init = true;
    while (__any_sync(kFullMask, addr < end_addr)) {
        if (need_init) {
            keccak_zero(a);
#pragma unroll
            for (int w = 0; w < 4; w++) a[w] = rho[w];
            a[4].lo = (b32 & 0xFFu) | ((b33 & 0xFFu) << 8) | (kSfxXof << 16);
            a[kRateShake128 - 1].hi ^= 0x80000000u;
            groups_left = group_limit;
            need_init = false;
        }
        keccak_f1600(a);
        const bool running = addr < end_addr;
        if (__any_sync(kFullMask, running && groups_left < 56)) {
            if (running && groups_left < 56) mask_groups(a, groups_left);
        }
        if (__all_sync(kFullMask, addr + 2 * 112 <= end_addr)) parse_block<false>(a, addr, end_addr);
        else parse_block<true>(a, addr, end_addr);
        groups_left -= 56;
        if (groups_left <= 0 && addr < end_addr) {
            b32 = (b32 + 1) & 0xFFu;
            b33 = (b33 + 1) & 0xFFu;
            addr = base;
            need_init = true;
        }
    }
}

#ifdef MLKEM_B200_EXPERIMENT
#define MLKEM_CHECK_SLOT_STORE(st, lim) \
    if ((st) + 512 < end_addr || (st) > (lim)) __trap();
#else
#define MLKEM_CHECK_SLOT_STORE(st, lim)
#endif
template <bool CHECKED>
__device__ __forceinline__ void parse_chunk3(const uint32_t w[7], uint32_t &addr, uint32_t end_addr) {
#ifndef MLKEM_B200_PARSE_ALU_ADDR
    const uint32_t one = c_pow2[0], two = c_pow2[1];
#endif
#pragma unroll
    for (int m = 0; m < 16; m++) {
        const int bit = 12 * m, wi = bit >> 5, sh = bit & 31;
        uint32_t t;
        if (sh == 20) t = w[wi];
        else if (sh < 20) t = shl_fma(w[wi], 20 - sh);
        else t = __funnelshift_r(w[wi], w[wi + 1], sh - 20);
        const bool ok = t < (kQ << 20);
        MLKEM_CHECK_SLOT_STORE(addr, CHECKED ? end_addr : end_addr - 2)
        asm volatile("st.shared.u16 [%0], %1;" ::"r"(addr), "h"((uint16_t)(t >> 20)) : "memory");
#ifndef MLKEM_B200_PARSE_ALU_ADDR
        if (CHECKED)
            asm volatile("{.reg .pred p; setp.lt.u32 p, %1, %2; setp.lt.and.u32 p, %0, %3, p; @p mad.lo.u32 %0, %4, %5, %0;}"
                         : "+r"(addr) : "r"(t), "r"(kQ << 20), "r"(end_addr), "r"(one), "r"(two));
        else
            asm volatile("{.reg .pred p; setp.lt.u32 p, %1, %2; @p mad.lo.u32 %0, %3, %4, %0;}" : "+r"(addr) : "r"(t), "r"(kQ << 20), "r"(one), "r"(two));
        (void)ok;
#else
        if (CHECKED) {
            if (ok && addr < end_addr) addr += 2;
        } else {
            if (ok) addr += 2;
        }
#endif
    }
}
template <bool CHECKED>
__device__ __forceinline__ void parse_block3(const Lane a[25], uint32_t &addr, uint32_t end_addr) {
#pragma unroll
    for (int ch = 0; ch < 7; ch++) {
        const uint32_t w[7] = {a[3 * ch].lo, a[3 * ch].hi, a[3 * ch + 1].lo, a[3 * ch + 1].hi, a[3 * ch + 2].lo, a[3 * ch + 2].hi, 0u};
        parse_chunk3<CHECKED>(w, addr, end_addr);
    }
}
__device__ __forceinline__ bool sample_ntt_three_blocks(const Lane rho[4], uint32_t b32, uint32_t b33, uint16_t *slot, int experiment = 0) {
    Lane a[25];
    const uint32_t base = (uint32_t)__cvta_generic_to_shared(slot), end_addr = base + 2 * kN;
    uint32_t addr = base;
    keccak_zero(a);
#pragma unroll
    for (int w = 0; w < 4; w++) a[w] = rho[w];
    a[4].lo = (b32 & 0xFFu) | ((b33 & 0xFFu) << 8) | (kSfxXof << 16);
    a[kRateShake128 - 1].hi ^= 0x80000000u;
#pragma unroll 1
    for (int blk = 0; blk < 3; blk++) {
        keccak_f1600(a);
#ifdef MLKEM_B200_EXPERIMENT
        if (experiment & 2) {
            addr += a[0].lo & 2;
            continue;
        }
#endif
        if (blk < 2) parse_block3<false>(a, addr, end_addr);
        else parse_block3<true>(a, addr, end_addr);
    }
    return addr >= end_addr;
}

enum MatvecMode { kModeKeyGen = 0, kModeEncrypt = 1, kModeEncryptCompare = 2 };

struct MatvecArgs {
    int n;
    int group_limit;
    const uint8_t *rho;
    size_t rho_stride;
    KeySel keys;
    const uint16_t *vec;
    size_t vec_stride;
    const uint16_t *add16;
    size_t add16_stride;
    const uint32_t *addc;
    size_t addc_stride;
    uint8_t *out;
    size_t out_stride;
    uint8_t *out2;
    size_t out2_stride;
    const uint8_t *cmp;
    uint32_t *flags;
    int *defer_list;
    int *defer_count;
#ifdef MLKEM_B200_EXPERIMENT
    int experiment;
#endif
};

constexpr int kMatvecWarpBytes = 512 + 384;
template <class P>
__host__ __device__ constexpr size_t matvec_slots_bytes() {
    return ((size_t)32 * P::K * kSlotWords * 4 + 15) & ~(size_t)15;
}
template <class P>
constexpr size_t matvec_smem_bytes() {
    return matvec_slots_bytes<P>() + (size_t)P::K * kMatvecWarpBytes + 32 * 4 + 32 * P::K;
}

struct MatvecLaneConsts {
    uint2 gam[4];
    LaneTwiddles tw;
    uint32_t pw;
};
template <int MODE>
__device__ __forceinline__ void matvec_load_consts(MatvecLaneConsts &c, int lane) {
#pragma unroll
    for (int r = 0; r < 4; r++) c.gam[r] = lane_gamma(lane + 32 * r);
    if (MODE != kModeKeyGen) load_lane_twiddles_inv<kFmaPipe>(c.tw, lane);
    c.pw = nibble_weight(lane & 7);
}
template <class P>
struct MatvecOperands {
    static constexpr int kCmpWords = (8 * P::DU + 31) / 32;
    uint32_t v[8 * P::K], cw[8], cmp[kCmpWords], ev[4];
};
template <class P, int MODE>
__device__ __forceinline__ void matvec_prefetch(MatvecOperands<P> &o, const MatvecArgs &g, int gg, int lane) {
    constexpr int K = P::K;
    if (gg < 0) return;
    const int item = gg / K, row = gg - item * K;
    const uint16_t *vec = g.vec + g.vec_stride * item;
#pragma unroll
    for (int j = 0; j < K; j++)
#pragma unroll
        for (int r = 0; r < 4; r++) {
            int t = lane + 32 * r;
            o.v[8 * j + 2 * r] = __ldg(vec + 256 * j + 2 * t);
            o.v[8 * j + 2 * r + 1] = __ldg(vec + 256 * j + 2 * t + 1);
        }
    if (MODE == kModeEncryptCompare) {
        const uint32_t *cw = reinterpret_cast<const uint32_t *>(g.cmp + g.out_stride * item + (size_t)P::C1ROW * row);
#pragma unroll
        for (int i = 0; i < MatvecOperands<P>::kCmpWords; i++) o.cmp[i] = (lane + 32 * i < 8 * P::DU) ? __ldg(cw + lane + 32 * i) : 0u;
    }
    if (MODE != kModeKeyGen) {
        const uint32_t *codes = g.addc + g.addc_stride * item + 32 * row + (lane >> 3);
#pragma unroll
        for (int r = 0; r < 8; r++) o.cw[r] = __ldg(codes + 4 * r);
    } else {
        const uint32_t *ev = reinterpret_cast<const uint32_t *>(g.add16 + g.add16_stride * item + 256 * row);
#pragma unroll
        for (int r = 0; r < 4; r++) o.ev[r] = __ldg(ev + lane + 32 * r);
    }
}

template <class P, int MODE>
__device__ __forceinline__ void matvec_row_tail(const MatvecArgs &g, int item, int row, uint32_t acc[8], const uint32_t cw8[8],
                                                const uint32_t *cmpw, const uint32_t ev4[4], uint16_t *scratch, uint8_t *stage, int lane,
                                                const LaneTwiddles &tw, uint32_t pw) {
    constexpr int kCmpWords = MatvecOperands<P>::kCmpWords;
    int nwords;
    if (MODE == kModeKeyGen) {
#pragma unroll
        for (int r = 0; r < 4; r++) {
            int t = lane + 32 * r;
            uint32_t e = ev4[r];
            uint32_t c0 = csubq(canon32(acc[2 * r]) + (e & 0xFFFFu)), c1 = csubq(canon32(acc[2 * r + 1]) + (e >> 16));
            uint32_t v = c0 | (c1 << 12);
            stage[3 * t] = (uint8_t)v;
            stage[3 * t + 1] = (uint8_t)(v >> 8);
            stage[3 * t + 2] = (uint8_t)(v >> 16);
        }
        nwords = 96;
    } else {
        uint32_t *sw = reinterpret_cast<uint32_t *>(scratch);
#pragma unroll
        for (int r = 0; r < 4; r++) {
            int t = lane + 32 * r;
            sw[sidx(2 * t) >> 1] = barrett32(acc[2 * r]) + barrett32(acc[2 * r + 1]) * 65536u;
        }
        __syncwarp();
        uint32_t x[8];
        load_scratch_C(x, scratch, lane);
        __syncwarp();
        intt_warp<kFmaPipe, false>(x, scratch, lane, tw);
#pragma unroll
        for (int r = 0; r < 8; r++) {
            uint32_t y = x[r] + nibble_fma(cw8[r], pw) + (kQ - 3);
            x[r] = compress_canon<P::DU>(canon_fma(y));
        }
        store_scratch_A(x, scratch, lane);
        __syncwarp();
        load_scratch_C(x, scratch, lane);
        pack8<P::DU>(x, stage + P::DU * lane);
        nwords = 8 * P::DU;
    }
    __syncwarp();
    const uint32_t *stw = reinterpret_cast<const uint32_t *>(stage);
    const size_t row_off = (MODE == kModeKeyGen ? 384 : P::C1ROW) * (size_t)row;
    if (MODE == kModeEncryptCompare) {
        uint32_t d = 0;
#pragma unroll
        for (int i = 0; i < kCmpWords; i++)
            if (lane + 32 * i < nwords) d |= stw[lane + 32 * i] ^ cmpw[i];
        d = __any_sync(kFullMask, d != 0) ? 1u : 0u;
        if (lane == 0) atomicOr(g.flags + item, d);
    } else {
        uint32_t *ow = reinterpret_cast<uint32_t *>(g.out + g.out_stride * item + row_off);
        for (int w = lane; w < nwords; w += 32) ow[w] = stw[w];
        if (MODE == kModeKeyGen && g.out2) {
            uint32_t *ow2 = reinterpret_cast<uint32_t *>(g.out2 + g.out2_stride * item + row_off);
            for (int w = lane; w < nwords; w += 32) ow2[w] = stw[w];
        }
    }
    __syncwarp();
}

template <class P, int MODE>
__device__ __forceinline__ void matvec_finish_rows(const MatvecArgs &g, uint32_t *s_slots, const int *s_gg, int lane, int warp,
                                                   const MatvecLaneConsts &lc, MatvecOperands<P> &nx) {
    constexpr int K = P::K;
    uint8_t *warp_area = reinterpret_cast<uint8_t *>(s_slots) + matvec_slots_bytes<P>() + warp * kMatvecWarpBytes;
    uint16_t *scratch = reinterpret_cast<uint16_t *>(warp_area);
    uint8_t *stage = warp_area + 512;
    const uint2 *gam = lc.gam;
    const LaneTwiddles &tw = lc.tw;
    const uint32_t pw = lc.pw;

    constexpr int kCmpWords = MatvecOperands<P>::kCmpWords;
#pragma unroll 1
    for (int grp = warp; grp < 32; grp += K) {
        const int gg = s_gg[grp];
        uint32_t v[8 * K], cw8[8], cmpw[kCmpWords], ev4[4];
#pragma unroll
        for (int i = 0; i < 8 * K; i++) v[i] = nx.v[i];
#pragma unroll
        for (int i = 0; i < 8; i++) cw8[i] = nx.cw[i];
#pragma unroll
        for (int i = 0; i < kCmpWords; i++) cmpw[i] = nx.cmp[i];
#pragma unroll
        for (int i = 0; i < 4; i++) ev4[i] = nx.ev[i];
        matvec_prefetch<P, MODE>(nx, g, grp + K < 32 ? s_gg[grp + K] : -1, lane);
        if (gg < 0) continue;
        const int item = gg / K, row = gg - item * K;
        const uint32_t slot0 = (uint32_t)__cvta_generic_to_shared(s_slots + kSlotWords * (grp * K));
        uint32_t acc[8];
#pragma unroll
        for (int r = 0; r < 8; r++) acc[r] = 0;
#pragma unroll
        for (int j = 0; j < K; j++) {
#pragma unroll
            for (int r = 0; r < 4; r++) {
                uint16_t a0, a1;
                const uint32_t ad = slot0 + 4 * (kSlotWords * j + lane + 32 * r);
                asm volatile("ld.shared.u16 %0, [%1];" : "=h"(a0) : "r"(ad));
                asm volatile("ld.shared.u16 %0, [%1+2];" : "=h"(a1) : "r"(ad));
                basemul_acc(acc[2 * r], acc[2 * r + 1], a0, a1, v[8 * j + 2 * r], v[8 * j + 2 * r + 1], gam[r]);
            }
        }
        matvec_row_tail<P, MODE>(g, item, row, acc, cw8, cmpw, ev4, scratch, stage, lane, tw, pw);
    }
}

template <class P>
__device__ __forceinline__ int *matvec_gg(uint32_t *s_slots) {
    return reinterpret_cast<int *>(reinterpret_cast<uint8_t *>(s_slots) + matvec_slots_bytes<P>() + P::K * kMatvecWarpBytes);
}

template <class P, int MODE>
__global__ void __launch_bounds__(32 * P::K) k_sample_matvec(MatvecArgs g) {
    constexpr int K = P::K;
    extern __shared__ __align__(16) uint32_t s_slots[];
    const int tid = threadIdx.x, lane = tid & 31, warp = tid >> 5;
    int *s_gg = matvec_gg<P>(s_slots);
    uint8_t *s_inc = reinterpret_cast<uint8_t *>(s_gg + 32);
    {
        const int grp = tid / K, col = tid - grp * K;
        const int gg = blockIdx.x * 32 + grp;
        const int item = gg / K, row = gg - item * K;
        const bool active = item < g.n;
        Lane rho[4];
#pragma unroll
        for (int w = 0; w < 4; w++) rho[w] = active ? load_lane(g.rho + g.rho_stride * key_row(g.keys, item) + 8 * w) : Lane{0u, 0u};
        const uint32_t b32 = MODE == kModeKeyGen ? col : row, b33 = MODE == kModeKeyGen ? row : col;
#ifdef MLKEM_B200_EXPERIMENT
        const bool complete = (g.experiment & 8) ? true
                                                 : sample_ntt_three_blocks(rho, b32, b33, reinterpret_cast<uint16_t *>(s_slots + kSlotWords * tid), g.experiment);
#else
        const bool complete = sample_ntt_three_blocks(rho, b32, b33, reinterpret_cast<uint16_t *>(s_slots + kSlotWords * tid));
#endif
        s_inc[tid] = active && !complete;
    }
    MatvecLaneConsts lc;
    matvec_load_consts<MODE>(lc, lane);
    MatvecOperands<P> nx;
    {
        const int gg = blockIdx.x * 32 + warp;
        matvec_prefetch<P, MODE>(nx, g, gg / K < g.n ? gg : -1, lane);
    }
    __syncthreads();
    {
        const int grp = warp + K * lane;
        if (grp < 32) {
            const int gg = blockIdx.x * 32 + grp;
            bool deferred = false;
#pragma unroll
            for (int j = 0; j < K; j++) deferred |= s_inc[grp * K + j] != 0;
            const bool active = gg / K < g.n;
            s_gg[grp] = (active && !deferred) ? gg : -1;
            if (active && deferred) g.defer_list[atomicAdd(g.defer_count, 1)] = gg;
        }
        __syncwarp();
    }
#ifdef MLKEM_B200_EXPERIMENT
    if (g.experiment & 1) return;
    if (g.experiment & 4) {
        matvec_finish_rows<P, MODE>(g, s_slots, s_gg, lane, warp, lc, nx);
        matvec_prefetch<P, MODE>(nx, g, s_gg[warp], lane);
    }
#endif
    matvec_finish_rows<P, MODE>(g, s_slots, s_gg, lane, warp, lc, nx);
}

template <class P, int MODE>
__global__ void __launch_bounds__(32 * P::K) k_sample_matvec_list(MatvecArgs g) {
    constexpr int K = P::K;
    extern __shared__ __align__(16) uint32_t s_slots[];
    const int tid = threadIdx.x, lane = tid & 31, warp = tid >> 5;
    int *s_gg = matvec_gg<P>(s_slots);
    MatvecLaneConsts lc;
    matvec_load_consts<MODE>(lc, lane);
    const int count = g.defer_list ? *g.defer_count : g.n * K;
    for (int base = blockIdx.x * 32; base < count; base += gridDim.x * 32) {
        {
            const int grp = tid / K, col = tid - grp * K;
            const int e = base + grp;
            const int gg = e < count ? (g.defer_list ? g.defer_list[e] : e) : -1;
            const bool active = gg >= 0;
            const int item = active ? gg / K : 0, row = gg - item * K;
            if (col == 0) s_gg[grp] = gg;
            Lane rho[4];
#pragma unroll
            for (int w = 0; w < 4; w++) rho[w] = active ? load_lane(g.rho + g.rho_stride * key_row(g.keys, item) + 8 * w) : Lane{0u, 0u};
            uint32_t b32 = MODE == kModeKeyGen ? col : row, b33 = MODE == kModeKeyGen ? row : col;
            sample_ntt_thread(rho, b32, b33, reinterpret_cast<uint16_t *>(s_slots + kSlotWords * tid), active, g.group_limit);
        }
        __syncthreads();
        MatvecOperands<P> nx;
        matvec_prefetch<P, MODE>(nx, g, s_gg[warp], lane);
        matvec_finish_rows<P, MODE>(g, s_slots, s_gg, lane, warp, lc, nx);
        __syncthreads();
    }
}


template <class P>
__global__ void __launch_bounds__(256) k_matrix_seeds(int n, const uint8_t *__restrict__ ek, size_t ek_stride, uint8_t *__restrict__ seeds) {
    constexpr int K = P::K;
    const int e = blockIdx.x * blockDim.x + threadIdx.x;
    if (e >= n * K * K) return;
    const int key = e / (K * K), rc = e - key * K * K, row = rc / K, col = rc - row * K;
    const uint8_t *rho = ek + ek_stride * key + 384 * K;
    uint8_t *out = seeds + 34 * (size_t)e;
    for (int b = 0; b < 32; b++) out[b] = rho[b];
    out[32] = (uint8_t)row;
    out[33] = (uint8_t)col;
}

__global__ void __launch_bounds__(256) k_scatter_rows(int n, int row_words, const uint8_t *__restrict__ src, size_t src_stride, KeySel slots,
                                                      uint8_t *__restrict__ dst, size_t dst_stride) {
    const size_t total = (size_t)n * row_words;
    for (size_t t = (size_t)blockIdx.x * blockDim.x + threadIdx.x; t < total; t += (size_t)gridDim.x * blockDim.x) {
        const int i = (int)(t / row_words), w = (int)(t - (size_t)i * row_words);
        const uint4 v = reinterpret_cast<const uint4 *>(src + src_stride * i)[w];
        reinterpret_cast<uint4 *>(dst + dst_stride * key_row(slots, i))[w] = v;
    }
}

__global__ void __launch_bounds__(kHashTPB) k_expand_seed(int n, const uint8_t *__restrict__ seed, unsigned long long first, uint32_t tag,
                                                          uint8_t *__restrict__ out0, uint8_t *__restrict__ out1) {
    const int j = blockIdx.x * blockDim.x + threadIdx.x;
    if (j >= n) return;
    const unsigned long long idx = first + (unsigned long long)j;
    Lane a[25];
    sponge_absorb_words<kRateSha3_256>(a, 6, kSfxXof, [&](int w) {
        if (w < 4) return load_lane(seed + 8 * w);
        return w == 4 ? Lane{(uint32_t)idx, (uint32_t)(idx >> 32)} : Lane{tag, 0u};
    });
#pragma unroll
    for (int w = 0; w < 4; w++) store_lane(out0 + 32 * (size_t)j + 8 * w, a[w]);
    if (out1) {
#pragma unroll
        for (int w = 0; w < 4; w++) store_lane(out1 + 32 * (size_t)j + 8 * w, a[4 + w]);
    }
}

#ifndef MLKEM_B200_MATTABLE_PREFETCH
#define MLKEM_B200_MATTABLE_PREFETCH 1
#endif
#ifndef MLKEM_B200_MATTABLE_BLOCKS
#define MLKEM_B200_MATTABLE_BLOCKS 1
#endif
template <class P, int MODE>
__global__ void __launch_bounds__(kMatTableTPB, MLKEM_B200_MATTABLE_BLOCKS) k_matvec_table(MatvecArgs g, const uint16_t *__restrict__ table) {
    static_assert(MODE != kModeKeyGen, "the table is kept in Encrypt order");
    constexpr int K = P::K, NW = kMatTableTPB / 32;
    __shared__ __align__(16) uint8_t s_warp[NW * kMatvecWarpBytes];
    const int lane = threadIdx.x & 31, warp = threadIdx.x >> 5;
    uint16_t *scratch = reinterpret_cast<uint16_t *>(s_warp + warp * kMatvecWarpBytes);
    uint8_t *stage = s_warp + warp * kMatvecWarpBytes + 512;
    MatvecLaneConsts lc;
    matvec_load_consts<MODE>(lc, lane);
    const int rows = g.n * K, stride = gridDim.x * NW;
    int gg = blockIdx.x * NW + warp;
    MatvecOperands<P> nx;
    if (MLKEM_B200_MATTABLE_PREFETCH) matvec_prefetch<P, MODE>(nx, g, gg < rows ? gg : -1, lane);
    constexpr int kCmpWords = MatvecOperands<P>::kCmpWords;
#pragma unroll 1
    for (; gg < rows; gg += stride) {
        if (!MLKEM_B200_MATTABLE_PREFETCH) matvec_prefetch<P, MODE>(nx, g, gg, lane);
        const int item = gg / K, row = gg - item * K;
        const uint32_t *arow = reinterpret_cast<const uint32_t *>(table + ((size_t)key_row(g.keys, item) * K + row) * K * 256);
        uint32_t aw[4 * K];
#pragma unroll
        for (int j = 0; j < K; j++)
#pragma unroll
            for (int r = 0; r < 4; r++) aw[4 * j + r] = __ldg(arow + 128 * j + lane + 32 * r);
        uint32_t v[8 * K], cw8[8], cmpw[kCmpWords], ev4[4];
#pragma unroll
        for (int i = 0; i < 8 * K; i++) v[i] = nx.v[i];
#pragma unroll
        for (int i = 0; i < 8; i++) cw8[i] = nx.cw[i];
#pragma unroll
        for (int i = 0; i < kCmpWords; i++) cmpw[i] = nx.cmp[i];
#pragma unroll
        for (int i = 0; i < 4; i++) ev4[i] = 0;
        if (MLKEM_B200_MATTABLE_PREFETCH) matvec_prefetch<P, MODE>(nx, g, gg + stride < rows ? gg + stride : -1, lane);
        uint32_t acc[8];
#pragma unroll
        for (int r = 0; r < 8; r++) acc[r] = 0;
#pragma unroll
        for (int j = 0; j < K; j++)
#pragma unroll
            for (int r = 0; r < 4; r++)
                basemul_acc(acc[2 * r], acc[2 * r + 1], aw[4 * j + r] & 0xFFFFu, aw[4 * j + r] >> 16, v[8 * j + 2 * r], v[8 * j + 2 * r + 1], lc.gam[r]);
        matvec_row_tail<P, MODE>(g, item, row, acc, cw8, cmpw, ev4, scratch, stage, lane, lc.tw, lc.pw);
    }
}

constexpr int kWarpTPB = 128;
#ifndef MLKEM_B200_PRIM_PIPE
#define MLKEM_B200_PRIM_PIPE false
#endif
constexpr bool kPrimPipe = MLKEM_B200_PRIM_PIPE;

struct EncVArgs {
    int n;
    const uint8_t *ek;
    size_t ek_stride;
    KeySel keys;
    const uint16_t *yhat;
    size_t yhat_stride;
    const uint32_t *addc;
    size_t addc_stride;
    const uint8_t *m;
    uint8_t *c;
    size_t c_stride;
    const uint8_t *cmp;
    uint32_t *flags;
};

__device__ __forceinline__ uint32_t smem_u32(const void *p) { return (uint32_t)__cvta_generic_to_shared(p); }
__device__ __forceinline__ void mbar_init(uint64_t *bar, int count) {
    asm volatile("mbarrier.init.shared::cta.b64 [%0], %1;" ::"r"(smem_u32(bar)), "r"(count) : "memory");
}
__device__ __forceinline__ void mbar_fence_init() { asm volatile("fence.mbarrier_init.release.cluster;" ::: "memory"); }
__device__ __forceinline__ void mbar_expect_tx(uint64_t *bar, uint32_t bytes) {
    asm volatile("mbarrier.arrive.expect_tx.shared::cta.b64 _, [%0], %1;" ::"r"(smem_u32(bar)), "r"(bytes) : "memory");
}
__device__ __forceinline__ void mbar_wait(uint64_t *bar, uint32_t parity) {
    asm volatile(
        "{\n"
        ".reg .pred p;\n"
        "WAIT_%=:\n"
        "mbarrier.try_wait.parity.shared::cta.b64 p, [%0], %1;\n"
        "@p bra DONE_%=;\n"
        "bra WAIT_%=;\n"
        "DONE_%=:\n"
        "}\n" ::"r"(smem_u32(bar)),
        "r"(parity)
        : "memory");
}
__device__ __forceinline__ void bulk_g2s(void *smem_dst, const void *gmem_src, uint32_t bytes, uint64_t *bar) {
    asm volatile("cp.async.bulk.shared::cluster.global.mbarrier::complete_tx::bytes [%0], [%1], %2, [%3];" ::"r"(smem_u32(smem_dst)),
                 "l"(gmem_src), "r"(bytes), "r"(smem_u32(bar))
                 : "memory");
}

#ifndef MLKEM_B200_ENCV_BLOCKS
#define MLKEM_B200_ENCV_BLOCKS 7
#endif
template <class P, bool COMPARE>
__global__ void __launch_bounds__(kWarpTPB, MLKEM_B200_ENCV_BLOCKS) k_encrypt_v(EncVArgs g) {
    constexpr int K = P::K, NW = kWarpTPB / 32;
    constexpr int kRowsBytes = 384 * K, kVecBytes = 512 * K, kBufBytes = kRowsBytes + kVecBytes + 16;
    __shared__ __align__(16) uint16_t s_scratch[NW * kScratchU16];
    __shared__ __align__(16) uint8_t s_in[NW * 2 * kBufBytes];
    __shared__ __align__(16) uint8_t s_stage[NW * 32 * P::DV];
    __shared__ __align__(8) uint64_t s_bar[NW * 2];
    const int lane = threadIdx.x & 31, warp = threadIdx.x >> 5;
    uint16_t *scratch = s_scratch + warp * kScratchU16;
    uint8_t *inbuf = s_in + warp * 2 * kBufBytes;
    uint8_t *stage = s_stage + warp * 32 * P::DV;
    uint64_t *bar = s_bar + 2 * warp;
    if (lane == 0) {
        mbar_init(bar, 1);
        mbar_init(bar + 1, 1);
        mbar_fence_init();
    }
    __syncwarp();
    uint2 gam[4];
#pragma unroll
    for (int i = 0; i < 4; i++) gam[i] = lane_gamma(4 * lane + i);
    LaneTwiddles tw;
    load_lane_twiddles_inv<kFmaPipe>(tw, lane);
    const uint32_t pw = nibble_weight(lane & 7);
    auto fetch = [&](int item, int b) {
        uint8_t *buf = inbuf + b * kBufBytes;
        mbar_expect_tx(bar + b, kRowsBytes + kVecBytes);
        bulk_g2s(buf, g.ek + g.ek_stride * key_row(g.keys, item), kRowsBytes, bar + b);
        bulk_g2s(buf + kRowsBytes, g.yhat + g.yhat_stride * item, kVecBytes, bar + b);
    };
    const int stride = gridDim.x * NW;
    int item = blockIdx.x * NW + warp, cur = 0;
    uint32_t phase = 0;
    if (item < g.n && lane == 0) fetch(item, 0);
    for (; item < g.n; item += stride, cur ^= 1) {
        if (item + stride < g.n && lane == 0) fetch(item + stride, cur ^ 1);
        mbar_wait(bar + cur, (phase >> cur) & 1u);
        phase ^= 1u << cur;
        const uint8_t *rows = inbuf + cur * kBufBytes;
        const uint16_t *yv = reinterpret_cast<const uint16_t *>(rows + kRowsBytes);
        const uint32_t *codes = g.addc + g.addc_stride * item + 32 * K;
        const uint32_t *mw = reinterpret_cast<const uint32_t *>(g.m + 32 * (size_t)item);
        uint32_t cw8[8], mw8[8];
#pragma unroll
        for (int r = 0; r < 8; r++) {
            cw8[r] = __ldg(codes + (lane >> 3) + 4 * r);
            mw8[r] = __ldg(mw + r);
        }
        uint32_t acc[8];
#pragma unroll
        for (int r = 0; r < 8; r++) acc[r] = 0;
#pragma unroll
        for (int j = 0; j < K; j++) {
            uint32_t t[8], y[8];
            unpack8<12>(rows + 384 * j, lane, t);
            unpack_pairs(*reinterpret_cast<const uint4 *>(yv + 256 * j + 8 * lane), y);
#pragma unroll
            for (int i = 0; i < 4; i++) basemul_acc(acc[2 * i], acc[2 * i + 1], t[2 * i], t[2 * i + 1], y[2 * i], y[2 * i + 1], gam[i]);
        }
        uint32_t x[8];
#pragma unroll
        for (int r = 0; r < 8; r++) x[r] = barrett32(acc[r]);
        intt_warp<kFmaPipe, false>(x, scratch, lane, tw);
#pragma unroll
        for (int r = 0; r < 8; r++) {
            uint32_t mu = ((mw8[r] >> lane) & 1u) * 1665u;
            x[r] = compress_resid<P::DV>(x[r] + nibble_fma(cw8[r], pw) + (kQ - 3) + mu);
        }
        store_scratch_A(x, scratch, lane);
        __syncwarp();
        load_scratch_C(x, scratch, lane);
        pack8<P::DV>(x, stage + P::DV * lane);
        __syncwarp();
        const uint32_t *stw = reinterpret_cast<const uint32_t *>(stage);
        const size_t off = (size_t)P::C1ROW * K;
        if (COMPARE) {
            const uint32_t *cw = reinterpret_cast<const uint32_t *>(g.cmp + g.c_stride * item + off);
            uint32_t d = 0;
            for (int w = lane; w < 8 * P::DV; w += 32) d |= stw[w] ^ __ldg(cw + w);
            d = __any_sync(kFullMask, d != 0) ? 1u : 0u;
            if (lane == 0) atomicOr(g.flags + item, d);
        } else {
            uint32_t *ow = reinterpret_cast<uint32_t *>(g.c + g.c_stride * item + off);
            for (int w = lane; w < 8 * P::DV; w += 32) ow[w] = stw[w];
        }
        __syncwarp();
    }
}

template <class P>
__global__ void __launch_bounds__(kWarpTPB) k_decrypt(int n, const uint8_t *__restrict__ dk, size_t dk_stride, KeySel keys,
                                                      const uint8_t *__restrict__ c, uint8_t *__restrict__ mout) {
    constexpr int K = P::K, NW = kWarpTPB / 32;
    constexpr int kSkBytes = 384 * K, kBufBytes = P::C + kSkBytes + 32;
    __shared__ __align__(16) uint16_t s_scratch[NW * kScratchU16];
    __shared__ __align__(16) uint8_t s_in[NW * 2 * kBufBytes];
    __shared__ __align__(8) uint64_t s_bar[NW * 2];
    const int lane = threadIdx.x & 31, warp = threadIdx.x >> 5;
    uint16_t *scratch = s_scratch + warp * kScratchU16;
    uint8_t *inbuf = s_in + warp * 2 * kBufBytes;
    uint64_t *bar = s_bar + 2 * warp;
    if (lane == 0) {
        mbar_init(bar, 1);
        mbar_init(bar + 1, 1);
        mbar_fence_init();
    }
    __syncwarp();
    uint2 gam[4];
#pragma unroll
    for (int i = 0; i < 4; i++) gam[i] = lane_gamma(4 * lane + i);
    LaneTwiddles tw, twi;
    load_lane_twiddles<kPrimPipe>(tw, lane);
    load_lane_twiddles_inv<kPrimPipe>(twi, lane);
    auto fetch = [&](int item, int b) {
        uint8_t *buf = inbuf + b * kBufBytes;
        mbar_expect_tx(bar + b, P::C + kSkBytes);
        bulk_g2s(buf, c + (size_t)P::C * item, P::C, bar + b);
        bulk_g2s(buf + P::C, dk + dk_stride * key_row(keys, item), kSkBytes, bar + b);
    };
    const int stride = gridDim.x * NW;
    int item = blockIdx.x * NW + warp, cur = 0;
    uint32_t phase = 0;
    if (item < n && lane == 0) fetch(item, 0);
    for (; item < n; item += stride, cur ^= 1) {
        if (item + stride < n && lane == 0) fetch(item + stride, cur ^ 1);
        mbar_wait(bar + cur, (phase >> cur) & 1u);
        phase ^= 1u << cur;
        const uint8_t *ct = inbuf + cur * kBufBytes, *sk = ct + P::C;
        uint32_t acc[8];
#pragma unroll
        for (int r = 0; r < 8; r++) acc[r] = 0;
        for (int i = 0; i < K; i++) {
            uint32_t x[8], sh[8];
            unpack8<P::DU>(ct + P::C1ROW * i, lane, x);
#pragma unroll
            for (int r = 0; r < 8; r++) x[r] = decompress<P::DU>(x[r]);
            store_scratch_C(x, scratch, lane);
            __syncwarp();
            load_scratch_A(x, scratch, lane);
            __syncwarp();
            ntt_warp<kPrimPipe>(x, scratch, lane, tw);
            unpack8<12>(sk + 384 * i, lane, sh);
#pragma unroll
            for (int p = 0; p < 4; p++) basemul_acc(acc[2 * p], acc[2 * p + 1], sh[2 * p], sh[2 * p + 1], x[2 * p], x[2 * p + 1], gam[p]);
        }
        uint32_t x[8];
#pragma unroll
        for (int r = 0; r < 8; r++) x[r] = kPrimPipe ? barrett32(acc[r]) : canon32(acc[r]);
        intt_warp<kPrimPipe>(x, scratch, lane, twi);
        uint32_t myword = 0;
#pragma unroll
        for (int r = 0; r < 8; r++) {
            uint32_t v = decompress<P::DV>(unpack1<P::DV>(ct + P::C1ROW * K, idxA(lane, r)));
            uint32_t w = csubq(v + kQ - x[r]);
            uint32_t word = __ballot_sync(kFullMask, compress_canon<1>(w) & 1u);
            if (lane == r) myword = word;
        }
        if (lane < 8) reinterpret_cast<uint32_t *>(mout + 32 * (size_t)item)[lane] = myword;
        __syncwarp();
    }
}

constexpr int kPrimTPB = 256;

__global__ void __launch_bounds__(kPrimTPB) k_ntt_batch(int n, const uint16_t *__restrict__ in, uint16_t *__restrict__ out) {
    __shared__ __align__(16) uint16_t s_scratch[(kPrimTPB / 32) * kScratchU16];
    const int lane = threadIdx.x & 31, warp = threadIdx.x >> 5;
    uint16_t *scratch = s_scratch + warp * kScratchU16;
    LaneTwiddles tw;
    load_lane_twiddles<kPrimPipe>(tw, lane);
    const long long stride = (long long)gridDim.x * (kPrimTPB / 32);
    long long p = (long long)blockIdx.x * (kPrimTPB / 32) + warp;
    uint32_t nxt[8];
    if (p < n) {
#pragma unroll
        for (int r = 0; r < 8; r++) nxt[r] = __ldg(in + 256 * p + idxA(lane, r));
    }
    for (; p < n; p += stride) {
        uint32_t x[8];
#pragma unroll
        for (int r = 0; r < 8; r++) x[r] = nxt[r] & 0xFFFu;
        if (p + stride < n) {
#pragma unroll
            for (int r = 0; r < 8; r++) nxt[r] = __ldg(in + 256 * (p + stride) + idxA(lane, r));
        }
        bool big = false;
#pragma unroll
        for (int r = 0; r < 8; r++) big |= x[r] >= kQ;
        if (__any_sync(kFullMask, big)) ntt_warp_exact(x, scratch, lane);
        else ntt_warp<kPrimPipe>(x, scratch, lane, tw);
        store_layoutC_global(x, lane, out + 256 * p);
    }
}
__global__ void __launch_bounds__(kPrimTPB) k_intt_batch(int n, const uint16_t *__restrict__ in, uint16_t *__restrict__ out) {
    __shared__ __align__(16) uint16_t s_scratch[(kPrimTPB / 32) * kScratchU16];
    const int lane = threadIdx.x & 31, warp = threadIdx.x >> 5;
    uint16_t *scratch = s_scratch + warp * kScratchU16;
    LaneTwiddles tw;
    load_lane_twiddles_inv<kPrimPipe>(tw, lane);
    const long long stride = (long long)gridDim.x * (kPrimTPB / 32);
    long long p = (long long)blockIdx.x * (kPrimTPB / 32) + warp;
    uint4 nxt = make_uint4(0, 0, 0, 0);
    if (p < n) nxt = __ldg(reinterpret_cast<const uint4 *>(in + 256 * p) + lane);
    for (; p < n; p += stride) {
        uint32_t x[8];
        unpack_pairs(nxt, x);
        if (p + stride < n) nxt = __ldg(reinterpret_cast<const uint4 *>(in + 256 * (p + stride)) + lane);
#pragma unroll
        for (int r = 0; r < 8; r++) x[r] &= 0xFFFu;
        intt_warp<kPrimPipe>(x, scratch, lane, tw);
        uint16_t *dst = out + 256 * p;
#pragma unroll
        for (int r = 0; r < 8; r++) dst[idxA(lane, r)] = (uint16_t)x[r];
    }
}
__global__ void __launch_bounds__(kPrimTPB) k_mulntt_batch(int n, const uint16_t *__restrict__ f, const uint16_t *__restrict__ gq,
                                                           uint16_t *__restrict__ h) {
    const int lane = threadIdx.x & 31, warp = threadIdx.x >> 5;
    uint2 gam[4];
#pragma unroll
    for (int r = 0; r < 4; r++) gam[r] = lane_gamma(lane + 32 * r);
    for (long long p = (long long)blockIdx.x * (kPrimTPB / 32) + warp; p < n; p += (long long)gridDim.x * (kPrimTPB / 32)) {
        const uint32_t *fw = reinterpret_cast<const uint32_t *>(f + 256 * p), *gw = reinterpret_cast<const uint32_t *>(gq + 256 * p);
        uint32_t *hw = reinterpret_cast<uint32_t *>(h + 256 * p);
#pragma unroll
        for (int r = 0; r < 4; r++) {
            int t = lane + 32 * r;
            uint32_t a = __ldg(fw + t), b = __ldg(gw + t), c0 = 0, c1 = 0;
            basemul_acc(c0, c1, a & 0xFFFu, (a >> 16) & 0xFFFu, b & 0xFFFu, (b >> 16) & 0xFFFu, gam[r]);
            hw[t] = canon32(c0) | (canon32(c1) << 16);
        }
    }
}

template <bool SUB>
__global__ void __launch_bounds__(kPrimTPB) k_poly_addsub(long long nvec, const uint4 *__restrict__ u, const uint4 *__restrict__ v,
                                                          uint4 *__restrict__ z) {
    for (long long i = (long long)blockIdx.x * blockDim.x + threadIdx.x; i < nvec; i += (long long)gridDim.x * blockDim.x) {
        const uint4 a4 = __ldg(u + i), b4 = __ldg(v + i);
        const uint32_t a[4] = {a4.x, a4.y, a4.z, a4.w}, b[4] = {b4.x, b4.y, b4.z, b4.w};
        uint32_t o[4];
#pragma unroll
        for (int k = 0; k < 4; k++) {
            uint32_t r[2];
#pragma unroll
            for (int h = 0; h < 2; h++) {
                const uint32_t x = (a[k] >> (16 * h)) & 0xFFFu, y = (b[k] >> (16 * h)) & 0xFFFu;
                r[h] = SUB ? ((x < y ? kQ - (y - x) : x - y) & 0xFFFu) : canon16(x + y);
            }
            o[k] = r[0] | (r[1] << 16);
        }
        z[i] = make_uint4(o[0], o[1], o[2], o[3]);
    }
}
__global__ void __launch_bounds__(kPrimTPB) k_vecmul_batch(int n, int k, const uint16_t *__restrict__ u, const uint16_t *__restrict__ v,
                                                           uint16_t *__restrict__ w) {
    const int lane = threadIdx.x & 31, warp = threadIdx.x >> 5;
    uint2 gam[4];
#pragma unroll
    for (int r = 0; r < 4; r++) gam[r] = lane_gamma(lane + 32 * r);
    for (long long p = (long long)blockIdx.x * (kPrimTPB / 32) + warp; p < n; p += (long long)gridDim.x * (kPrimTPB / 32)) {
        uint32_t acc[8];
#pragma unroll
        for (int r = 0; r < 8; r++) acc[r] = 0;
        for (int j = 0; j < k; j++) {
            const uint32_t *uw = reinterpret_cast<const uint32_t *>(u + 256 * (p * k + j)), *vw = reinterpret_cast<const uint32_t *>(v + 256 * (p * k + j));
#pragma unroll
            for (int r = 0; r < 4; r++) {
                const uint32_t a = __ldg(uw + lane + 32 * r), b = __ldg(vw + lane + 32 * r);
                uint32_t c0 = 0, c1 = 0;
                basemul_acc(c0, c1, a & 0xFFFu, (a >> 16) & 0xFFFu, b & 0xFFFu, (b >> 16) & 0xFFFu, gam[r]);
                acc[2 * r] += canon32(c0);
                acc[2 * r + 1] += canon32(c1);
            }
        }
        uint32_t *ww = reinterpret_cast<uint32_t *>(w + 256 * p);
#pragma unroll
        for (int r = 0; r < 4; r++) ww[lane + 32 * r] = canon16(acc[2 * r]) | (canon16(acc[2 * r + 1]) << 16);
    }
}

__global__ void __launch_bounds__(128) k_sample_ntt_batch(int n, const uint8_t *__restrict__ seeds, uint16_t *__restrict__ out,
                                                          uint8_t *__restrict__ seeds_after, int group_limit) {
    extern __shared__ __align__(16) uint32_t s_slots[];
    const int tid = threadIdx.x, lane = tid & 31, warp = tid >> 5;
    const int item = blockIdx.x * 128 + tid;
    const bool active = item < n;
    Lane rho[4];
    uint32_t b32 = 0, b33 = 0;
    if (active) {
        const uint8_t *s = seeds + 34 * (size_t)item;
#pragma unroll
        for (int w = 0; w < 4; w++) {
            uint32_t lo = 0, hi = 0;
#pragma unroll
            for (int b = 0; b < 4; b++) {
                lo |= (uint32_t)s[8 * w + b] << (8 * b);
                hi |= (uint32_t)s[8 * w + 4 + b] << (8 * b);
            }
            rho[w] = Lane{lo, hi};
        }
        b32 = s[32];
        b33 = s[33];
    } else {
#pragma unroll
        for (int w = 0; w < 4; w++) rho[w] = Lane{0u, 0u};
    }
    sample_ntt_thread(rho, b32, b33, reinterpret_cast<uint16_t *>(s_slots + kSlotWords * tid), active, group_limit);
    if (active && seeds_after) {
        uint8_t *sa = seeds_after + 34 * (size_t)item;
        const uint8_t *s = seeds + 34 * (size_t)item;
        for (int b = 0; b < 32; b++) sa[b] = s[b];
        sa[32] = (uint8_t)b32;
        sa[33] = (uint8_t)b33;
    }
    __syncwarp();
    for (int t = 0; t < 32; t++) {
        int it = blockIdx.x * 128 + warp * 32 + t;
        if (it >= n) break;
        const uint32_t *src = s_slots + kSlotWords * (warp * 32 + t);
        uint32_t *dst = reinterpret_cast<uint32_t *>(out + 256 * (size_t)it);
#pragma unroll
        for (int r = 0; r < 4; r++) dst[lane + 32 * r] = src[lane + 32 * r];
    }
}

template <int ETA>
__global__ void __launch_bounds__(kPrimTPB) k_cbd_batch(int n, const uint8_t *__restrict__ in, uint16_t *__restrict__ out) {
    const int lane = threadIdx.x & 31, warp = threadIdx.x >> 5;
    for (long long p = (long long)blockIdx.x * (kPrimTPB / 32) + warp; p < n; p += (long long)gridDim.x * (kPrimTPB / 32)) {
        const uint8_t *src = in + (size_t)64 * ETA * p;
        uint32_t *dst = reinterpret_cast<uint32_t *>(out + 256 * p);
#pragma unroll
        for (int r = 0; r < 4; r++) {
            int t = lane + 32 * r;
            uint32_t c[2];
#pragma unroll
            for (int h = 0; h < 2; h++) {
                int bit = 2 * ETA * (2 * t + h);
                uint32_t w = (uint32_t)src[bit >> 3] | ((uint32_t)src[min((bit >> 3) + 1, 64 * ETA - 1)] << 8);
                w >>= (bit & 7);
                uint32_t x = __popc(w & ((1u << ETA) - 1u)), y = __popc((w >> ETA) & ((1u << ETA) - 1u));
                c[h] = x >= y ? x - y : kQ - (y - x);
            }
            dst[t] = c[0] | (c[1] << 16);
        }
    }
}

template <int ETA, int RATE = kRateShake128>
__global__ void __launch_bounds__(kNoiseTPB) k_prf_cbd_batch(int n, const uint8_t *__restrict__ seeds, const uint8_t *__restrict__ nonces,
                                                             uint16_t *__restrict__ out) {
    __shared__ uint32_t s_codes[kNoiseTPB * 33];
    const int item = blockIdx.x * kNoiseTPB + threadIdx.x;
    const int lane = threadIdx.x & 31, warp = threadIdx.x >> 5;
    Lane seed[4];
#pragma unroll
    for (int w = 0; w < 4; w++) seed[w] = item < n ? load_lane(seeds + 32 * (size_t)item + 8 * w) : Lane{0u, 0u};
    uint32_t nonce = item < n ? nonces[item] : 0u;
    uint32_t *mine = s_codes + 33 * threadIdx.x;
    prf_cbd_codes<ETA, RATE>(seed, nonce, [&](int w, uint32_t v) { mine[w] = v; });
    __syncwarp();
    for (int t = 0; t < 32; t++) {
        int it = blockIdx.x * kNoiseTPB + warp * 32 + t;
        if (it >= n) break;
        const uint32_t *codes = s_codes + 33 * (warp * 32 + t);
        uint32_t *dst = reinterpret_cast<uint32_t *>(out + 256 * (size_t)it);
#pragma unroll
        for (int r = 0; r < 4; r++) {
            int tt = lane + 32 * r;
            uint32_t wd = codes[tt >> 2] >> (8 * (tt & 3));
            dst[tt] = noise_code_to_coeff(wd & 15u) | (noise_code_to_coeff((wd >> 4) & 15u) << 16);
        }
    }
}

template <int D, bool COMPRESS>
__global__ void __launch_bounds__(kPrimTPB) k_encode_batch(int n, const uint16_t *__restrict__ in, uint8_t *__restrict__ out) {
    __shared__ __align__(16) uint8_t s_stage[(kPrimTPB / 32) * 32 * D];
    const int lane = threadIdx.x & 31, warp = threadIdx.x >> 5;
    uint8_t *stage = s_stage + warp * 32 * D;
    const long long stride = (long long)gridDim.x * (kPrimTPB / 32);
    long long p = (long long)blockIdx.x * (kPrimTPB / 32) + warp;
    uint4 nxt = make_uint4(0, 0, 0, 0);
    if (p < n) nxt = __ldg(reinterpret_cast<const uint4 *>(in + 256 * p) + lane);
    for (; p < n; p += stride) {
        uint4 q4 = nxt;
        if (p + stride < n) nxt = __ldg(reinterpret_cast<const uint4 *>(in + 256 * (p + stride)) + lane);
        uint32_t w[4] = {q4.x, q4.y, q4.z, q4.w}, v[8];
#pragma unroll
        for (int i = 0; i < 8; i++) {
            uint32_t c = (w[i >> 1] >> (16 * (i & 1))) & 0xFFFu;
            v[i] = (COMPRESS ? compress<D>(c) : c) & ((1u << D) - 1u);
        }
        pack8<D>(v, stage + D * lane);
        __syncwarp();
        const uint4 *sv = reinterpret_cast<const uint4 *>(stage);
        uint4 *ov = reinterpret_cast<uint4 *>(out + (size_t)32 * D * p);
        for (int i = lane; i < 2 * D; i += 32) ov[i] = sv[i];
        __syncwarp();
    }
}
template <int D, bool DECOMPRESS>
__global__ void __launch_bounds__(kPrimTPB) k_decode_batch(int n, const uint8_t *__restrict__ in, uint16_t *__restrict__ out) {
    __shared__ __align__(16) uint8_t s_stage[(kPrimTPB / 32) * 32 * D + 16];
    const int lane = threadIdx.x & 31, warp = threadIdx.x >> 5;
    uint8_t *stage = s_stage + warp * 32 * D;
    for (long long p = (long long)blockIdx.x * (kPrimTPB / 32) + warp; p < n; p += (long long)gridDim.x * (kPrimTPB / 32)) {
        const uint4 *iv = reinterpret_cast<const uint4 *>(in + (size_t)32 * D * p);
        uint4 *sv = reinterpret_cast<uint4 *>(stage);
        for (int i = lane; i < 2 * D; i += 32) sv[i] = __ldg(iv + i);
        __syncwarp();
        uint32_t v[8];
        unpack8<D>(stage, lane, v);
#pragma unroll
        for (int i = 0; i < 8; i++) v[i] = DECOMPRESS ? decompress<D>(v[i]) : v[i];
        reinterpret_cast<uint4 *>(out + 256 * p)[lane] =
            make_uint4(v[0] | (v[1] << 16), v[2] | (v[3] << 16), v[4] | (v[5] << 16), v[6] | (v[7] << 16));
        __syncwarp();
    }
}
template <int D, bool DECOMPRESS>
__global__ void __launch_bounds__(kPrimTPB) k_compress_batch(long long nvec, const uint4 *__restrict__ in, uint4 *__restrict__ out) {
    for (long long i = (long long)blockIdx.x * blockDim.x + threadIdx.x; i < nvec; i += (long long)gridDim.x * blockDim.x) {
        uint4 q4 = __ldg(in + i);
        uint32_t w[4] = {q4.x, q4.y, q4.z, q4.w};
#pragma unroll
        for (int k = 0; k < 4; k++) {
            uint32_t lo = w[k] & 0xFFFu, hi = (w[k] >> 16) & 0xFFFu;
            if (DECOMPRESS) {
                lo = decompress<D>(lo & ((1u << D) - 1u));
                hi = decompress<D>(hi & ((1u << D) - 1u));
            } else {
                lo = compress<D>(lo);
                hi = compress<D>(hi);
            }
            w[k] = lo | (hi << 16);
        }
        out[i] = make_uint4(w[0], w[1], w[2], w[3]);
    }
}

}
```

Baseline: 33.73 million.

## Replace first five NTT layers with int8 tensor-core MMA matrix transform

Folds the first five forward NTT layers (and the last five inverse layers plus the final scaling) into a precomputed 32x32 transform matrix. The matrix is applied per 32-coefficient block using mma.sync m16n8k32 s8 instructions, with coefficients split into 6/7-bit limbs and recombined by Barrett reduction. This removes two shared-memory transposes and most of the butterfly ALU work per polynomial. Lane layouts for noise sampling, matvec tails and decrypt are rewritten to the new MMA output ordering, and message extraction now packs bits per lane instead of using ballots. The risk is extra limb-splitting and MMA latency, plus layout-mismatch bugs across the many call sites.

```diff
diff --git a/crystals-kyber_b200/csrc/mlkem_b200.cu b/crystals-kyber_b200/csrc/mlkem_b200.cu
--- a/crystals-kyber_b200/csrc/mlkem_b200.cu
+++ b/crystals-kyber_b200/csrc/mlkem_b200.cu
@@ -106,10 +106,6 @@
         t.gamma32[i] = shoup_pair32(t.gamma[i].x);
         t.zeta32[i] = shoup_pair32(t.zeta[i].x);
     }
-    t.zeta_inv_last[0] = shoup_pair((t.zeta[1].x * 3303u) % kQ);
-    t.zeta_inv_last[1] = shoup_pair(3303u);
-    t.zeta_inv_last32[0] = shoup_pair32(t.zeta_inv_last[0].x);
-    t.zeta_inv_last32[1] = shoup_pair32(3303u);
     uint8_t lfsr = 1;
     for (int round = 0; round < 24; round++) {
         unsigned long long c = 0;
@@ -121,6 +117,51 @@
         }
         rc[round] = make_uint2((unsigned)c, (unsigned)(c >> 32));
     }
+}
+
+void transform_matrix(const TwiddleTables &t, bool inverse, unsigned M[32][32]) {
+    for (int col = 0; col < 32; col++) {
+        unsigned v[32] = {};
+        v[col] = 1;
+        int k = inverse ? 31 : 1;
+        for (int step = 0; step < 5; step++) {
+            const int len = inverse ? 1 << step : 16 >> step;
+            for (int start = 0; start < 32; start += 2 * len) {
+                const unsigned z = t.zeta[inverse ? k-- : k++].x;
+                for (int j = start; j < start + len; j++) {
+                    if (inverse) {
+                        const unsigned a = v[j];
+                        v[j] = (a + v[j + len]) % kQ;
+                        v[j + len] = z * ((v[j + len] + kQ - a) % kQ) % kQ;
+                    } else {
+                        const unsigned tz = z * v[j + len] % kQ;
+                        v[j + len] = (v[j] + kQ - tz) % kQ;
+                        v[j] = (v[j] + tz) % kQ;
+                    }
+                }
+            }
+        }
+        for (int row = 0; row < 32; row++) M[row][col] = inverse ? v[row] * 3303u % kQ : v[row];
+    }
+}
+void build_mma_fragments(const unsigned M[32][32], uint4 frag[4][2][32]) {
+    const int rho[4] = {0, 2, 1, 3};
+    for (int w = 0; w < 4; w++)
+        for (int tile = 0; tile < 2; tile++)
+            for (int lane = 0; lane < 32; lane++) {
+                const int g = lane >> 2, tq = lane & 3;
+                unsigned reg[4];
+                for (int i = 0; i < 4; i++) {
+                    const int p = 16 * tile + g + 8 * (i & 1), h = i >> 1;
+                    reg[i] = 0;
+                    for (int j = 0; j < 4; j++) {
+                        const int m = 4 * (4 * h + rho[j]) + tq;
+                        const unsigned e = w < 2 ? M[p][m] : 64u * M[p][m] % kQ;
+                        reg[i] |= ((w & 1) ? (e & 63u) : (e >> 6)) << (8 * j);
+                    }
+                }
+                frag[w][tile][lane] = make_uint4(reg[0], reg[1], reg[2], reg[3]);
+            }
 }
 
 struct DeviceCtx {
@@ -208,6 +249,14 @@
             CU(cudaMemcpyToSymbol(c_tw, &t, sizeof t));
             CU(cudaMemcpyToSymbol(g_tw, &t, sizeof t));
             CU(cudaMemcpyToSymbol(c_keccak_rc, rc, sizeof rc));
+            unsigned M[32][32];
+            uint4 frag[4][2][32];
+            transform_matrix(t, false, M);
+            build_mma_fragments(M, frag);
+            CU(cudaMemcpyToSymbol(g_ntt_frag, frag, sizeof frag));
+            transform_matrix(t, true, M);
+            build_mma_fragments(M, frag);
+            CU(cudaMemcpyToSymbol(g_intt_frag, frag, sizeof frag));
             uint32_t pow2[32];
             for (int k = 0; k < 32; k++) pow2[k] = 1u << k;
             CU(cudaMemcpyToSymbol(c_pow2, pow2, sizeof pow2));
diff --git a/crystals-kyber_b200/csrc/mlkem_device.cuh b/crystals-kyber_b200/csrc/mlkem_device.cuh
--- a/crystals-kyber_b200/csrc/mlkem_device.cuh
+++ b/crystals-kyber_b200/csrc/mlkem_device.cuh
@@ -10,11 +10,9 @@
 
 struct TwiddleTables {
     uint2 zeta[128];
-    uint2 zeta_inv_last[2];
     uint2 gamma[128];
     uint2 gamma32[128];
     uint2 zeta32[128];
-    uint2 zeta_inv_last32[2];
 };
 __constant__ TwiddleTables c_tw;
 __device__ TwiddleTables g_tw;
@@ -296,18 +294,6 @@
 #pragma unroll
     for (int i = 0; i < 2; i++) t.z2[i] = lane_z<FMA>(64 + 2 * lane + i);
 }
-template <bool FMA = false>
-__device__ __forceinline__ void load_lane_twiddles_inv(LaneTwiddles &t, int lane) {
-    int g = lane >> 2;
-    t.z16 = lane_z<FMA>(15 - g);
-#pragma unroll
-    for (int i = 0; i < 2; i++) t.z8[i] = lane_z<FMA>(31 - (2 * g + i));
-#pragma unroll
-    for (int i = 0; i < 4; i++) t.z4[i] = lane_z<FMA>(63 - (4 * g + i));
-#pragma unroll
-    for (int i = 0; i < 2; i++) t.z2[i] = lane_z<FMA>(127 - (2 * lane + i));
-}
-
 __device__ __forceinline__ void store_scratch_A(const uint32_t x[8], uint16_t *s, int lane) {
 #pragma unroll
     for (int r = 0; r < 8; r++) s[sidx(idxA(lane, r))] = (uint16_t)x[r];
@@ -345,38 +331,99 @@
     a = a + t;
 }
 
-template <bool FMA = false>
-__device__ __forceinline__ void ntt_warp(uint32_t x[8], uint16_t *scratch, int lane, const LaneTwiddles &tw) {
-#pragma unroll
-    for (int r = 0; r < 4; r++) ct_bfly<FMA>(x[r], x[r + 4], uniform_z<FMA>(1));
+__device__ uint4 g_ntt_frag[4][2][32];
+__device__ uint4 g_intt_frag[4][2][32];
+__device__ __forceinline__ int laneM(int lane) { return 8 * (lane & 3) + (lane >> 2); }
+__device__ __forceinline__ int idxM(int lane, int r) { return laneM(lane) + 32 * r; }
+__device__ __forceinline__ void load_scratch_M(uint32_t x[8], const uint16_t *s, int lane) {
+#pragma unroll
+    for (int r = 0; r < 8; r++) x[r] = s[sidx(idxM(lane, r))];
+}
+struct TwiddlesC {
+    uint2 z4, z2[2];
+};
+template <bool FMA = false>
+__device__ __forceinline__ void load_twiddles_c(TwiddlesC &t, int lane) {
+    t.z4 = lane_z<FMA>(32 + lane);
+#pragma unroll
+    for (int i = 0; i < 2; i++) t.z2[i] = lane_z<FMA>(64 + 2 * lane + i);
+}
+
+template <bool FMA = false>
+__device__ __forceinline__ void load_twiddles_c_inv(TwiddlesC &t, int lane) {
+    t.z4 = lane_z<FMA>(63 - lane);
+#pragma unroll
+    for (int i = 0; i < 2; i++) t.z2[i] = lane_z<FMA>(127 - (2 * lane + i));
+}
+
+__device__ __forceinline__ void mma_s8(int32_t d[4], uint4 a, uint32_t b0, uint32_t b1, const int32_t c[4]) {
+    asm("mma.sync.aligned.m16n8k32.row.col.s32.s8.s8.s32 {%0, %1, %2, %3}, {%4, %5, %6, %7}, {%8, %9}, {%10, %11, %12, %13};"
+        : "=r"(d[0]), "=r"(d[1]), "=r"(d[2]), "=r"(d[3])
+        : "r"(a.x), "r"(a.y), "r"(a.z), "r"(a.w), "r"(b0), "r"(b1), "r"(c[0]), "r"(c[1]), "r"(c[2]), "r"(c[3]));
+}
+__device__ __forceinline__ void split_limbs(const uint32_t x[8], uint32_t bh[2], uint32_t bl[2]) {
+#pragma unroll
+    for (int h = 0; h < 2; h++) {
+        const uint32_t p01 = __byte_perm(x[4 * h], x[4 * h + 1], 0x5410), p23 = __byte_perm(x[4 * h + 2], x[4 * h + 3], 0x5410);
+        bl[h] = __byte_perm(p01 & 0x003F003Fu, p23 & 0x003F003Fu, 0x6240);
+        bh[h] = __byte_perm((p01 >> 6) & 0x007F007Fu, (p23 >> 6) & 0x007F007Fu, 0x6240);
+    }
+}
+template <bool FMA>
+__device__ __forceinline__ void ntt_warp_finish(const int32_t a64[8], const int32_t a1[8], uint32_t x[8], uint16_t *scratch, int lane,
+                                                const TwiddlesC &tw) {
+    uint32_t *sw = reinterpret_cast<uint32_t *>(scratch);
+#pragma unroll
+    for (int k = 0; k < 4; k++) {
+        const uint32_t y0 = barrett32((uint32_t)a64[2 * k] * c_pow2[6] + (uint32_t)a1[2 * k]);
+        const uint32_t y1 = barrett32((uint32_t)a64[2 * k + 1] * c_pow2[6] + (uint32_t)a1[2 * k + 1]);
+        sw[32 * k + lane] = y0 + y1 * 65536u;
+    }
+    __syncwarp();
+    unpack_pairs(reinterpret_cast<const uint4 *>(sw)[lane], x);
+    __syncwarp();
+#pragma unroll
+    for (int r = 0; r < 4; r++) ct_bfly<FMA>(x[r], x[r + 4], tw.z4);
 #pragma unroll
     for (int h = 0; h < 2; h++)
 #pragma unroll
-        for (int r = 0; r < 2; r++) ct_bfly<FMA>(x[4 * h + r], x[4 * h + r + 2], uniform_z<FMA>(2 + h));
-#pragma unroll
-    for (int h = 0; h < 4; h++) ct_bfly<FMA>(x[2 * h], x[2 * h + 1], uniform_z<FMA>(4 + h));
-    store_scratch_A(x, scratch, lane);
-    __syncwarp();
-    load_scratch_B(x, scratch, lane);
-    __syncwarp();
-#pragma unroll
-    for (int r = 0; r < 4; r++) ct_bfly<FMA>(x[r], x[r + 4], tw.z16);
-#pragma unroll
-    for (int h = 0; h < 2; h++)
-#pragma unroll
-        for (int r = 0; r < 2; r++) ct_bfly<FMA>(x[4 * h + r], x[4 * h + r + 2], tw.z8[h]);
-#pragma unroll
-    for (int h = 0; h < 4; h++) ct_bfly<FMA>(x[2 * h], x[2 * h + 1], tw.z4[h]);
-    store_scratch_B(x, scratch, lane);
-    __syncwarp();
-    load_scratch_C(x, scratch, lane);
-    __syncwarp();
-#pragma unroll
-    for (int h = 0; h < 2; h++)
-#pragma unroll
         for (int r = 0; r < 2; r++) ct_bfly<FMA>(x[4 * h + r], x[4 * h + r + 2], tw.z2[h]);
 #pragma unroll
     for (int r = 0; r < 8; r++) x[r] = FMA ? canon_fma(x[r]) : canon16(x[r]);
+}
+__device__ __forceinline__ void mma_two_limbs(const uint4 (*frag)[2][32], const uint32_t x[8], int lane, int32_t a64[8], int32_t a1[8]) {
+    uint32_t bh[2], bl[2];
+    split_limbs(x, bh, bl);
+    const int32_t zero[4] = {0, 0, 0, 0};
+#pragma unroll
+    for (int T = 0; T < 2; T++) {
+        const uint4 mh = __ldg(&frag[0][T][lane]), ml = __ldg(&frag[1][T][lane]);
+        const uint4 m64h = __ldg(&frag[2][T][lane]), m64l = __ldg(&frag[3][T][lane]);
+        mma_s8(a64 + 4 * T, m64h, bh[0], bh[1], zero);
+        mma_s8(a64 + 4 * T, mh, bl[0], bl[1], a64 + 4 * T);
+        mma_s8(a1 + 4 * T, m64l, bh[0], bh[1], zero);
+        mma_s8(a1 + 4 * T, ml, bl[0], bl[1], a1 + 4 * T);
+    }
+}
+template <bool FMA = false>
+__device__ __forceinline__ void ntt_warp(uint32_t x[8], uint16_t *scratch, int lane, const TwiddlesC &tw) {
+    int32_t a64[8], a1[8];
+    mma_two_limbs(g_ntt_frag, x, lane, a64, a1);
+    ntt_warp_finish<FMA>(a64, a1, x, scratch, lane, tw);
+}
+__device__ __forceinline__ uint32_t pack_s8_codes(uint32_t c0, uint32_t c1, uint32_t c2, uint32_t c3) {
+    return (c0 + c2 * 256u + c1 * 65536u + c3 * 16777216u + 0x7D7D7D7Du) ^ 0x80808080u;
+}
+template <bool FMA = false>
+__device__ __forceinline__ void ntt_warp_s8(const uint32_t b[2], uint32_t x[8], uint16_t *scratch, int lane, const TwiddlesC &tw) {
+    const int32_t zero[4] = {0, 0, 0, 0}, bias[4] = {98 * (int32_t)kQ, 98 * (int32_t)kQ, 98 * (int32_t)kQ, 98 * (int32_t)kQ};
+    int32_t a64[8], a1[8];
+#pragma unroll
+    for (int T = 0; T < 2; T++) {
+        mma_s8(a64 + 4 * T, __ldg(&g_ntt_frag[0][T][lane]), b[0], b[1], zero);
+        mma_s8(a1 + 4 * T, __ldg(&g_ntt_frag[1][T][lane]), b[0], b[1], bias);
+    }
+    ntt_warp_finish<FMA>(a64, a1, x, scratch, lane, tw);
 }
 
 __device__ __forceinline__ void ct_bfly_exact(uint32_t &a, uint32_t &b, uint2 z) {
@@ -425,49 +472,28 @@
 }
 
 template <bool FMA = false, bool CANON = true>
-__device__ __forceinline__ void intt_warp(uint32_t x[8], uint16_t *scratch, int lane, const LaneTwiddles &tw) {
+__device__ __forceinline__ void intt_warp(uint32_t x[8], uint16_t *scratch, int lane, const TwiddlesC &tw) {
 #pragma unroll
     for (int h = 0; h < 2; h++)
 #pragma unroll
         for (int r = 0; r < 2; r++) gs_bfly<FMA>(x[4 * h + r], x[4 * h + r + 2], tw.z2[h], (FMA ? 3 : 2) * kQ);
-    store_scratch_C(x, scratch, lane);
-    __syncwarp();
-    load_scratch_B(x, scratch, lane);
-    __syncwarp();
-#pragma unroll
-    for (int h = 0; h < 4; h++) {
-        gs_bfly<FMA>(x[2 * h], x[2 * h + 1], tw.z4[h], (FMA ? 5 : 3) * kQ);
-        x[2 * h] = FMA ? barrett32(x[2 * h]) : barrett16(x[2 * h]);
-    }
-#pragma unroll
-    for (int h = 0; h < 2; h++)
-#pragma unroll
-        for (int r = 0; r < 2; r++) gs_bfly<FMA>(x[4 * h + r], x[4 * h + r + 2], tw.z8[h], 2 * kQ);
-#pragma unroll
-    for (int r = 0; r < 4; r++) gs_bfly<FMA>(x[r], x[r + 4], tw.z16, 4 * kQ);
-    store_scratch_B(x, scratch, lane);
-    __syncwarp();
-    load_scratch_A(x, scratch, lane);
-    __syncwarp();
-#pragma unroll
-    for (int h = 0; h < 4; h++) {
-        gs_bfly<FMA>(x[2 * h], x[2 * h + 1], uniform_z<FMA>(7 - h), 8 * kQ);
-        x[2 * h] = FMA ? barrett32(x[2 * h]) : barrett16(x[2 * h]);
-    }
-#pragma unroll
-    for (int h = 0; h < 2; h++)
-#pragma unroll
-        for (int r = 0; r < 2; r++) gs_bfly<FMA>(x[4 * h + r], x[4 * h + r + 2], uniform_z<FMA>(3 - h), 2 * kQ);
-    const uint2 zs = FMA ? c_tw.zeta_inv_last32[1] : c_tw.zeta_inv_last[1], zl = FMA ? c_tw.zeta_inv_last32[0] : c_tw.zeta_inv_last[0];
 #pragma unroll
     for (int r = 0; r < 4; r++) {
-        uint32_t t = x[r];
-        x[r] = mulz<FMA>(t + x[r + 4], zs);
-        x[r + 4] = mulz<FMA>(x[r + 4] - t + 4 * kQ, zl);
-        if (CANON) {
-            x[r] = csubq(x[r]);
-            x[r + 4] = csubq(x[r + 4]);
-        }
+        gs_bfly<FMA>(x[r], x[r + 4], tw.z4, (FMA ? 5 : 3) * kQ);
+        x[r] = FMA ? barrett32(x[r]) : barrett16(x[r]);
+    }
+    uint32_t *sw = reinterpret_cast<uint32_t *>(scratch);
+    reinterpret_cast<uint4 *>(sw)[lane] = pack_pairs(x);
+    __syncwarp();
+#pragma unroll
+    for (int r = 0; r < 8; r++) x[r] = scratch[idxM(lane, r)];
+    __syncwarp();
+    int32_t a64[8], a1[8];
+    mma_two_limbs(g_intt_frag, x, lane, a64, a1);
+#pragma unroll
+    for (int i = 0; i < 8; i++) {
+        x[i] = barrett32((uint32_t)a64[i] * c_pow2[6] + (uint32_t)a1[i]);
+        if (CANON) x[i] = csubq(x[i]);
     }
 }
 
diff --git a/crystals-kyber_b200/csrc/mlkem_kernels.cuh b/crystals-kyber_b200/csrc/mlkem_kernels.cuh
--- a/crystals-kyber_b200/csrc/mlkem_kernels.cuh
+++ b/crystals-kyber_b200/csrc/mlkem_kernels.cuh
@@ -441,17 +441,20 @@
         __syncwarp();
         const int lane = threadIdx.x & 31, warp = threadIdx.x >> 5;
         uint16_t *scratch = s_scratch + warp * kScratchU16;
-        LaneTwiddles tw;
-        load_lane_twiddles<kFmaPipe>(tw, lane);
-        const uint32_t pw = nibble_weight(lane & 7);
+        TwiddlesC tw;
+        load_twiddles_c<kFmaPipe>(tw, lane);
+        const int lm = laneM(lane);
+        const uint32_t pw = nibble_weight(lm & 7);
         for (int t = 0; t < 32; t++) {
             int it = blockIdx.x * kNoiseTPB + warp * 32 + t;
             if (it >= n) break;
-            const uint32_t *codes = s_codes + 33 * (warp * 32 + t) + (lane >> 3);
-            uint32_t x[8];
-#pragma unroll
-            for (int r = 0; r < 8; r++) x[r] = nibble_fma(codes[4 * r], pw) + (kQ - 3);
-            ntt_warp<kFmaPipe>(x, scratch, lane, tw);
+            const uint32_t *codes = s_codes + 33 * (warp * 32 + t) + (lm >> 3);
+            uint32_t c[8], b[2], x[8];
+#pragma unroll
+            for (int r = 0; r < 8; r++) c[r] = nibble_fma(codes[4 * r], pw);
+#pragma unroll
+            for (int h = 0; h < 2; h++) b[h] = pack_s8_codes(c[4 * h], c[4 * h + 1], c[4 * h + 2], c[4 * h + 3]);
+            ntt_warp_s8<kFmaPipe>(b, x, scratch, lane, tw);
             store_layoutC_global(x, lane, out16 + out16_stride * it + 256 * p);
             if (p < enc12_polys) {
                 uint32_t *row = reinterpret_cast<uint32_t *>(enc12 + enc12_stride * it + 384 * p) + 3 * lane;
@@ -647,20 +650,21 @@
 
 struct MatvecLaneConsts {
     uint2 gam[4];
-    LaneTwiddles tw;
-    uint32_t pw;
+    TwiddlesC tw;
+    uint32_t pw[2];
 };
 template <int MODE>
 __device__ __forceinline__ void matvec_load_consts(MatvecLaneConsts &c, int lane) {
 #pragma unroll
     for (int r = 0; r < 4; r++) c.gam[r] = lane_gamma(lane + 32 * r);
-    if (MODE != kModeKeyGen) load_lane_twiddles_inv<kFmaPipe>(c.tw, lane);
-    c.pw = nibble_weight(lane & 7);
+    if (MODE != kModeKeyGen) load_twiddles_c_inv<kFmaPipe>(c.tw, lane);
+    c.pw[0] = nibble_weight(2 * (lane & 3));
+    c.pw[1] = nibble_weight(2 * (lane & 3) + 1);
 }
 template <class P>
 struct MatvecOperands {
     static constexpr int kCmpWords = (8 * P::DU + 31) / 32;
-    uint32_t v[8 * P::K], cw[8], cmp[kCmpWords], ev[4];
+    uint32_t v[8 * P::K], cw[4], cmp[kCmpWords], ev[4];
 };
 template <class P, int MODE>
 __device__ __forceinline__ void matvec_prefetch(MatvecOperands<P> &o, const MatvecArgs &g, int gg, int lane) {
@@ -682,9 +686,9 @@
         for (int i = 0; i < MatvecOperands<P>::kCmpWords; i++) o.cmp[i] = (lane + 32 * i < 8 * P::DU) ? __ldg(cw + lane + 32 * i) : 0u;
     }
     if (MODE != kModeKeyGen) {
-        const uint32_t *codes = g.addc + g.addc_stride * item + 32 * row + (lane >> 3);
-#pragma unroll
-        for (int r = 0; r < 8; r++) o.cw[r] = __ldg(codes + 4 * r);
+        const uint32_t *codes = g.addc + g.addc_stride * item + 32 * row + (lane >> 2);
+#pragma unroll
+        for (int r = 0; r < 4; r++) o.cw[r] = __ldg(codes + 8 * r);
     } else {
         const uint32_t *ev = reinterpret_cast<const uint32_t *>(g.add16 + g.add16_stride * item + 256 * row);
 #pragma unroll
@@ -693,9 +697,9 @@
 }
 
 template <class P, int MODE>
-__device__ __forceinline__ void matvec_row_tail(const MatvecArgs &g, int item, int row, uint32_t acc[8], const uint32_t cw8[8],
+__device__ __forceinline__ void matvec_row_tail(const MatvecArgs &g, int item, int row, uint32_t acc[8], const uint32_t cw4[4],
                                                 const uint32_t *cmpw, const uint32_t ev4[4], uint16_t *scratch, uint8_t *stage, int lane,
-                                                const LaneTwiddles &tw, uint32_t pw) {
+                                                const TwiddlesC &tw, const uint32_t pw[2]) {
     constexpr int kCmpWords = MatvecOperands<P>::kCmpWords;
     int nwords;
     if (MODE == kModeKeyGen) {
@@ -723,13 +727,14 @@
         __syncwarp();
         intt_warp<kFmaPipe, false>(x, scratch, lane, tw);
 #pragma unroll
-        for (int r = 0; r < 8; r++) {
-            uint32_t y = x[r] + nibble_fma(cw8[r], pw) + (kQ - 3);
-            x[r] = compress_canon<P::DU>(canon_fma(y));
-        }
-        store_scratch_A(x, scratch, lane);
+        for (int i = 0; i < 8; i++) {
+            uint32_t y = x[i] + nibble_fma(cw4[i >> 1], pw[i & 1]) + (kQ - 3);
+            x[i] = compress_canon<P::DU>(canon_fma(y));
+        }
+#pragma unroll
+        for (int r = 0; r < 4; r++) sw[32 * r + lane] = x[2 * r] + x[2 * r + 1] * 65536u;
         __syncwarp();
-        load_scratch_C(x, scratch, lane);
+        unpack_pairs(reinterpret_cast<const uint4 *>(sw)[lane], x);
         pack8<P::DU>(x, stage + P::DU * lane);
         nwords = 8 * P::DU;
     }
@@ -762,18 +767,18 @@
     uint16_t *scratch = reinterpret_cast<uint16_t *>(warp_area);
     uint8_t *stage = warp_area + 512;
     const uint2 *gam = lc.gam;
-    const LaneTwiddles &tw = lc.tw;
-    const uint32_t pw = lc.pw;
+    const TwiddlesC &tw = lc.tw;
+    const uint32_t *pw = lc.pw;
 
     constexpr int kCmpWords = MatvecOperands<P>::kCmpWords;
 #pragma unroll 1
     for (int grp = warp; grp < 32; grp += K) {
         const int gg = s_gg[grp];
-        uint32_t v[8 * K], cw8[8], cmpw[kCmpWords], ev4[4];
+        uint32_t v[8 * K], cw4[4], cmpw[kCmpWords], ev4[4];
 #pragma unroll
         for (int i = 0; i < 8 * K; i++) v[i] = nx.v[i];
 #pragma unroll
-        for (int i = 0; i < 8; i++) cw8[i] = nx.cw[i];
+        for (int i = 0; i < 4; i++) cw4[i] = nx.cw[i];
 #pragma unroll
         for (int i = 0; i < kCmpWords; i++) cmpw[i] = nx.cmp[i];
 #pragma unroll
@@ -796,7 +801,7 @@
                 basemul_acc(acc[2 * r], acc[2 * r + 1], a0, a1, v[8 * j + 2 * r], v[8 * j + 2 * r + 1], gam[r]);
             }
         }
-        matvec_row_tail<P, MODE>(g, item, row, acc, cw8, cmpw, ev4, scratch, stage, lane, tw, pw);
+        matvec_row_tail<P, MODE>(g, item, row, acc, cw4, cmpw, ev4, scratch, stage, lane, tw, pw);
     }
 }
 
@@ -964,11 +969,11 @@
         for (int j = 0; j < K; j++)
 #pragma unroll
             for (int r = 0; r < 4; r++) aw[4 * j + r] = __ldg(arow + 128 * j + lane + 32 * r);
-        uint32_t v[8 * K], cw8[8], cmpw[kCmpWords], ev4[4];
+        uint32_t v[8 * K], cw4[4], cmpw[kCmpWords], ev4[4];
 #pragma unroll
         for (int i = 0; i < 8 * K; i++) v[i] = nx.v[i];
 #pragma unroll
-        for (int i = 0; i < 8; i++) cw8[i] = nx.cw[i];
+        for (int i = 0; i < 4; i++) cw4[i] = nx.cw[i];
 #pragma unroll
         for (int i = 0; i < kCmpWords; i++) cmpw[i] = nx.cmp[i];
 #pragma unroll
@@ -982,7 +987,7 @@
 #pragma unroll
             for (int r = 0; r < 4; r++)
                 basemul_acc(acc[2 * r], acc[2 * r + 1], aw[4 * j + r] & 0xFFFFu, aw[4 * j + r] >> 16, v[8 * j + 2 * r], v[8 * j + 2 * r + 1], lc.gam[r]);
-        matvec_row_tail<P, MODE>(g, item, row, acc, cw8, cmpw, ev4, scratch, stage, lane, lc.tw, lc.pw);
+        matvec_row_tail<P, MODE>(g, item, row, acc, cw4, cmpw, ev4, scratch, stage, lane, lc.tw, lc.pw);
     }
 }
 
@@ -1060,9 +1065,9 @@
     uint2 gam[4];
 #pragma unroll
     for (int i = 0; i < 4; i++) gam[i] = lane_gamma(4 * lane + i);
-    LaneTwiddles tw;
-    load_lane_twiddles_inv<kFmaPipe>(tw, lane);
-    const uint32_t pw = nibble_weight(lane & 7);
+    TwiddlesC tw;
+    load_twiddles_c_inv<kFmaPipe>(tw, lane);
+    const uint32_t pw[2] = {nibble_weight(2 * (lane & 3)), nibble_weight(2 * (lane & 3) + 1)};
     auto fetch = [&](int item, int b) {
         uint8_t *buf = inbuf + b * kBufBytes;
         mbar_expect_tx(bar + b, kRowsBytes + kVecBytes);
@@ -1081,12 +1086,11 @@
         const uint16_t *yv = reinterpret_cast<const uint16_t *>(rows + kRowsBytes);
         const uint32_t *codes = g.addc + g.addc_stride * item + 32 * K;
         const uint32_t *mw = reinterpret_cast<const uint32_t *>(g.m + 32 * (size_t)item);
-        uint32_t cw8[8], mw8[8];
-#pragma unroll
-        for (int r = 0; r < 8; r++) {
-            cw8[r] = __ldg(codes + (lane >> 3) + 4 * r);
-            mw8[r] = __ldg(mw + r);
-        }
+        uint32_t cw4[4], mw8[8];
+#pragma unroll
+        for (int r = 0; r < 8; r++) mw8[r] = __ldg(mw + r);
+#pragma unroll
+        for (int r = 0; r < 4; r++) cw4[r] = __ldg(codes + 8 * r + (lane >> 2));
         uint32_t acc[8];
 #pragma unroll
         for (int r = 0; r < 8; r++) acc[r] = 0;
@@ -1103,13 +1107,17 @@
         for (int r = 0; r < 8; r++) x[r] = barrett32(acc[r]);
         intt_warp<kFmaPipe, false>(x, scratch, lane, tw);
 #pragma unroll
-        for (int r = 0; r < 8; r++) {
-            uint32_t mu = ((mw8[r] >> lane) & 1u) * 1665u;
-            x[r] = compress_resid<P::DV>(x[r] + nibble_fma(cw8[r], pw) + (kQ - 3) + mu);
-        }
-        store_scratch_A(x, scratch, lane);
+        for (int i = 0; i < 8; i++) {
+            const int r = i >> 1, e = i & 1;
+            const uint32_t w = (lane & 16) ? mw8[2 * r + 1] : mw8[2 * r];
+            uint32_t mu = ((w >> ((2 * lane + e) & 31)) & 1u) * 1665u;
+            x[i] = compress_resid<P::DV>(x[i] + nibble_fma(cw4[r], pw[e]) + (kQ - 3) + mu);
+        }
+        uint32_t *sw = reinterpret_cast<uint32_t *>(scratch);
+#pragma unroll
+        for (int r = 0; r < 4; r++) sw[32 * r + lane] = x[2 * r] + x[2 * r + 1] * 65536u;
         __syncwarp();
-        load_scratch_C(x, scratch, lane);
+        unpack_pairs(reinterpret_cast<const uint4 *>(sw)[lane], x);
         pack8<P::DV>(x, stage + P::DV * lane);
         __syncwarp();
         const uint32_t *stw = reinterpret_cast<const uint32_t *>(stage);
@@ -1149,9 +1157,9 @@
     uint2 gam[4];
 #pragma unroll
     for (int i = 0; i < 4; i++) gam[i] = lane_gamma(4 * lane + i);
-    LaneTwiddles tw, twi;
-    load_lane_twiddles<kPrimPipe>(tw, lane);
-    load_lane_twiddles_inv<kPrimPipe>(twi, lane);
+    TwiddlesC tw, twi;
+    load_twiddles_c<kPrimPipe>(tw, lane);
+    load_twiddles_c_inv<kPrimPipe>(twi, lane);
     auto fetch = [&](int item, int b) {
         uint8_t *buf = inbuf + b * kBufBytes;
         mbar_expect_tx(bar + b, P::C + kSkBytes);
@@ -1177,7 +1185,7 @@
             for (int r = 0; r < 8; r++) x[r] = decompress<P::DU>(x[r]);
             store_scratch_C(x, scratch, lane);
             __syncwarp();
-            load_scratch_A(x, scratch, lane);
+            load_scratch_M(x, scratch, lane);
             __syncwarp();
             ntt_warp<kPrimPipe>(x, scratch, lane, tw);
             unpack8<12>(sk + 384 * i, lane, sh);
@@ -1188,15 +1196,16 @@
 #pragma unroll
         for (int r = 0; r < 8; r++) x[r] = kPrimPipe ? barrett32(acc[r]) : canon32(acc[r]);
         intt_warp<kPrimPipe>(x, scratch, lane, twi);
-        uint32_t myword = 0;
-#pragma unroll
-        for (int r = 0; r < 8; r++) {
-            uint32_t v = decompress<P::DV>(unpack1<P::DV>(ct + P::C1ROW * K, idxA(lane, r)));
-            uint32_t w = csubq(v + kQ - x[r]);
-            uint32_t word = __ballot_sync(kFullMask, compress_canon<1>(w) & 1u);
-            if (lane == r) myword = word;
-        }
-        if (lane < 8) reinterpret_cast<uint32_t *>(mout + 32 * (size_t)item)[lane] = myword;
+        uint32_t *sw = reinterpret_cast<uint32_t *>(scratch);
+#pragma unroll
+        for (int r = 0; r < 4; r++) sw[32 * r + lane] = x[2 * r] + x[2 * r + 1] * 65536u;
+        __syncwarp();
+        unpack_pairs(reinterpret_cast<const uint4 *>(sw)[lane], x);
+        uint32_t v[8], byte = 0;
+        unpack8<P::DV>(ct + P::C1ROW * K, lane, v);
+#pragma unroll
+        for (int r = 0; r < 8; r++) byte |= (compress_canon<1>(csubq(decompress<P::DV>(v[r]) + kQ - x[r])) & 1u) << r;
+        mout[32 * (size_t)item + lane] = (uint8_t)byte;
         __syncwarp();
     }
 }
@@ -1207,14 +1216,14 @@
     __shared__ __align__(16) uint16_t s_scratch[(kPrimTPB / 32) * kScratchU16];
     const int lane = threadIdx.x & 31, warp = threadIdx.x >> 5;
     uint16_t *scratch = s_scratch + warp * kScratchU16;
-    LaneTwiddles tw;
-    load_lane_twiddles<kPrimPipe>(tw, lane);
+    TwiddlesC tw;
+    load_twiddles_c<kPrimPipe>(tw, lane);
     const long long stride = (long long)gridDim.x * (kPrimTPB / 32);
     long long p = (long long)blockIdx.x * (kPrimTPB / 32) + warp;
     uint32_t nxt[8];
     if (p < n) {
 #pragma unroll
-        for (int r = 0; r < 8; r++) nxt[r] = __ldg(in + 256 * p + idxA(lane, r));
+        for (int r = 0; r < 8; r++) nxt[r] = __ldg(in + 256 * p + idxM(lane, r));
     }
     for (; p < n; p += stride) {
         uint32_t x[8];
@@ -1222,13 +1231,18 @@
         for (int r = 0; r < 8; r++) x[r] = nxt[r] & 0xFFFu;
         if (p + stride < n) {
 #pragma unroll
-            for (int r = 0; r < 8; r++) nxt[r] = __ldg(in + 256 * (p + stride) + idxA(lane, r));
+            for (int r = 0; r < 8; r++) nxt[r] = __ldg(in + 256 * (p + stride) + idxM(lane, r));
         }
         bool big = false;
 #pragma unroll
         for (int r = 0; r < 8; r++) big |= x[r] >= kQ;
-        if (__any_sync(kFullMask, big)) ntt_warp_exact(x, scratch, lane);
-        else ntt_warp<kPrimPipe>(x, scratch, lane, tw);
+        if (__any_sync(kFullMask, big)) {
+#pragma unroll
+            for (int r = 0; r < 8; r++) x[r] = __ldg(in + 256 * p + idxA(lane, r)) & 0xFFFu;
+            ntt_warp_exact(x, scratch, lane);
+        } else {
+            ntt_warp<kPrimPipe>(x, scratch, lane, tw);
+        }
         store_layoutC_global(x, lane, out + 256 * p);
     }
 }
@@ -1236,8 +1250,8 @@
     __shared__ __align__(16) uint16_t s_scratch[(kPrimTPB / 32) * kScratchU16];
     const int lane = threadIdx.x & 31, warp = threadIdx.x >> 5;
     uint16_t *scratch = s_scratch + warp * kScratchU16;
-    LaneTwiddles tw;
-    load_lane_twiddles_inv<kPrimPipe>(tw, lane);
+    TwiddlesC tw;
+    load_twiddles_c_inv<kPrimPipe>(tw, lane);
     const long long stride = (long long)gridDim.x * (kPrimTPB / 32);
     long long p = (long long)blockIdx.x * (kPrimTPB / 32) + warp;
     uint4 nxt = make_uint4(0, 0, 0, 0);
@@ -1249,9 +1263,9 @@
 #pragma unroll
         for (int r = 0; r < 8; r++) x[r] &= 0xFFFu;
         intt_warp<kPrimPipe>(x, scratch, lane, tw);
-        uint16_t *dst = out + 256 * p;
-#pragma unroll
-        for (int r = 0; r < 8; r++) dst[idxA(lane, r)] = (uint16_t)x[r];
+        uint32_t *dst = reinterpret_cast<uint32_t *>(out + 256 * p);
+#pragma unroll
+        for (int r = 0; r < 4; r++) dst[32 * r + lane] = x[2 * r] | (x[2 * r + 1] << 16);
     }
 }
 __global__ void __launch_bounds__(kPrimTPB) k_mulntt_batch(int n, const uint16_t *__restrict__ f, const uint16_t *__restrict__ gq,
```

After: 34.09 million, median of 6. 1.1% higher.
